# zouyunkai/MedicalSemSeg

Measured on AMD Instinct MI355X. Metric: 96^3 vols/sec fwd+bwd (train), higher is better.
Workload: dtype bf16; 1 GPU; UNet base (MONAI BasicUNet 32-32-64-128-256-32) 1->3cls, 96^3 patches, DiceCE + AdamW, per-GPU batch 2; global_batch=2, parallelism=dp1, grad_sync=none (single rank)

## Files before the change

### include/msseg.h

```cpp
#ifndef MSSEG_H_
#define MSSEG_H_

#include <stddef.h>
#include <stdint.h>

#ifdef __cplusplus
extern "C" {
#endif

#define MSSEG_ABI_VERSION 1

#define MSSEG_OK 0
#define MSSEG_EINVAL (-1)
#define MSSEG_ELAUNCH (-2)
#define MSSEG_EWORKSPACE (-3)

#define MSSEG_F32 0
#define MSSEG_BF16 1

typedef void* msseg_stream_t;

int msseg_abi_version(void);
const char* msseg_last_error(void);
int msseg_num_cus(void);
// ... 2 lines not shown
int msseg_ktimer_reset(void);
int msseg_ktimer_count(void);
int msseg_ktimer_get(int i, char* name, int cap, float* ms);

size_t msseg_packed_weight_bytes(int M, int T, int K, int cout_block, int dtype);
int msseg_pack_weights(const float* src, void* dst, int dtype, int M, int M0, int T, int K, int K0,
                       long long s_m1, long long s_m0, long long s_t, long long s_k1, long long s_k0,
                       int flip, int cout_block, msseg_stream_t stream);
typedef struct msseg_pack_job {
    const float* src;
    void* dst;
    long long s_m1, s_m0, s_t, s_k1, s_k0;
    long long total;
    int M, M0, T, K, K0, flip, cout_block, nkb;
} msseg_pack_job;
int msseg_pack_weights_batch(const msseg_pack_job* jobs_dev, int njobs, long long max_total, long long sum_total, int dtype,
                             msseg_stream_t stream);
int msseg_cout_block(int M);
int msseg_conv3d_k3_cout_block(int N, int D, int H, int W, int Cout);
int msseg_conv3d_k3_variant(int N, int D, int H, int W, int Cout);
int msseg_conv3d_k3_kernel(int N, int D, int H, int W, int Cin, int Cout, int dtype);

int msseg_conv3d_k3_fwd(const void* x, long long ldx, const void* wp, const float* bias, void* y, long long ldy,
                        int N, int D, int H, int W, int Cin, int Cout, float* stats ,
                        void* scratch, size_t scratch_bytes, int dtype, msseg_stream_t stream);
int msseg_conv3d_k3_fwd_accumulate(const void* x, long long ldx, const void* wp, void* y, long long ldy, int N, int D, int H,
                                   int W, int Cin, int Cout, float* stats, void* scratch, size_t scratch_bytes, int dtype,
                                   msseg_stream_t stream);
int msseg_conv3d_k3_dgrad_inbwd(const void* dy, long long lddy, const void* wp, void* da, long long ldda, int N, int D,
                                int H, int W, int Cin, int Cout, const void* yraw, long long ldyraw, const void* act,
                                long long ldact, const float* fwd_stats, float slope, float eps, float* red,
                                float* dgamma, float* dbeta, int accumulate, void* scratch, size_t scratch_bytes,
                                int dtype, msseg_stream_t stream);
int msseg_conv3d_k3s2_fwd(const void* x, long long ldx, const void* wp, const float* bias, void* y, long long ldy,
                          int N, int ID, int IH, int IW, int Cin, int Cout, int dtype, msseg_stream_t stream);
int msseg_zero_stuff2(const void* dy, long long lddy, void* out, long long ldo, int N, int OD, int OH, int OW, int ID,
                      int IH, int IW, int C, int dtype, msseg_stream_t stream);
int msseg_conv3d_stem_fwd(const void* x, long long ldx, const void* wp, const float* bias, void* y, long long ldy,
                          int N, int D, int H, int W, int Cout, float* stats, void* scratch, size_t scratch_bytes,
                          int dtype, msseg_stream_t stream);
int msseg_conv3d_stem_k1_fwd(const void* x, long long ldx, const void* wp, const float* bias, void* y, long long ldy,
                             int N, int D, int H, int W, int Cout, float* stats, void* scratch, size_t scratch_bytes,
                             int dtype, msseg_stream_t stream);
int msseg_conv3d_stem_norm_fwd(const void* x, long long ldx, const void* wp, const float* bias, const float* stats,
                               const float* gamma, const float* beta, float eps, float slope, void* y, long long ldy, int N,
                               int D, int H, int W, int Cout, int dtype, msseg_stream_t stream);
int msseg_conv3d_k1_fwd(const void* x, long long ldx, const void* wp, const float* bias, void* y, long long ldy,
                        long long NV, int Cin, int Cout, int dtype, msseg_stream_t stream);
int msseg_conv3d_k1_head_fwd(const void* x, long long ldx, const float* w, const float* bias, void* y, long long ldy,
                             long long NV, int Cin, int Cout, int dtype, msseg_stream_t stream);
int msseg_conv3d_k1_head_dgrad_inbwd(const void* dy, long long lddy, const float* w, void* da, long long ldda, int N,
                                     long long S, int C, int Cout, const void* yraw, long long ldyraw,
                                     const float* fwd_stats, const float* gamma, const float* beta, float slope, float eps,
                                     float* red, float* dgamma, float* dbeta, int accumulate, void* scratch,
                                     size_t scratch_bytes, int dtype, msseg_stream_t stream);
int msseg_conv3d_k1_head_norm_fwd(const void* x, long long ldx, const float* stats, const float* gamma, const float* beta,
                                  float slope, float eps, const float* w, const float* bias, void* y, long long ldy, int N,
                                  long long S, int Cin, int Cout, int dtype, msseg_stream_t stream);
int msseg_conv3d_k1_head_bwd_fused(const void* dy, long long lddy, const float* w, void* da, long long ldda, int N,
                                   long long S, int C, int Cout, const void* yraw, long long ldyraw, const float* fwd_stats,
                                   const float* gamma, const float* beta, float slope, float eps, float* red, float* dgamma,
                                   float* dbeta, int accumulate, float* dw, int dw_accumulate, void* scratch,
                                   size_t scratch_bytes, int dtype, msseg_stream_t stream);

int msseg_conv3d_gather_fwd(const void* x, long long ldx, const void* wp, const float* bias, void* y, long long ldy,
                            int N, int ID, int IH, int IW, int Cin, int Cout, int k, int s, int p, int dtype,
                            msseg_stream_t stream);
int msseg_deconv_k2s2_fwd(const void* x, long long ldx, const void* wp, const float* bias, void* y, long long ldy,
                          int N, int D, int H, int W, int Cin, int Cout, int dtype, msseg_stream_t stream);
int msseg_deconv_k2s2_bwd_data(const void* dy, long long lddy, const void* wp, void* dx, long long lddx,
                               int N, int D, int H, int W, int Cin, int Cout, int dtype, msseg_stream_t stream);
int msseg_deconv_k4s4_fwd(const void* x, long long ldx, const void* wp, const float* bias, void* y, long long ldy,
                          int N, int D, int H, int W, int Cin, int Cout, int dtype, msseg_stream_t stream);
// ... 74 lines not shown
int msseg_interp_trilinear_bwd(const void* dy, long long lddy, void* dx, long long lddx, int N, int ID, int IH, int IW, int OD,
                               int OH, int OW, int C, void* workspace, size_t workspace_bytes, int dtype, msseg_stream_t stream);
int msseg_kv_attention_fwd(const void* q, const void* kv, void* o, float* lse, int B, int N, int M, int heads, int head_dim,
                           float scale, int dtype, msseg_stream_t stream);
size_t msseg_kv_attention_bwd_workspace_bytes(int B, int N, int M, int heads, int head_dim);
int msseg_kv_attention_bwd(const void* q, const void* kv, const void* o, const float* lse, const void* dout, void* dq, void* dkv,
                           int B, int N, int M, int heads, int head_dim, float scale, void* workspace, size_t workspace_bytes,
                           int dtype, msseg_stream_t stream);
int msseg_scale_channels(const void* x, const float* scale, void* y, int N, long long S, int C, int dtype, msseg_stream_t stream);

size_t msseg_reduce_scratch_bytes(void);
int msseg_channel_stats(const void* x, long long ldx, float* stats, int N, long long S, int C, void* scratch,
                        size_t scratch_bytes, int dtype, msseg_stream_t stream);
int msseg_instnorm_act_fwd(const void* x, long long ldx, const float* stats, const float* gamma, const float* beta,
                           const void* residual, long long ldr, void* y, long long ldy, int N, long long S, int C,
                           float eps, float slope, int dtype, msseg_stream_t stream);
int msseg_instnorm_act_pool_fwd(const void* x, long long ldx, const float* stats, const float* gamma, const float* beta,
                                void* y, long long ldy, void* pooled, long long ldp, int N, int D, int H, int W, int C,
                                float eps, float slope, int dtype, msseg_stream_t stream);
int msseg_instnorm_act_poolbwd_reduce(const void* x, long long ldx, const float* stats, const float* gamma,
                                      const float* beta, const void* skip, long long lds, const void* g, long long ldg,
                                      void* da, long long ldda, float* red, float* dgamma, float* dbeta, int accumulate,
                                      int N, int D, int H, int W, int C, float eps, float slope, void* scratch,
                                      size_t scratch_bytes, int dtype, msseg_stream_t stream);
int msseg_instnorm_act_bwd_reduce(const void* x, long long ldx, const float* stats, const float* gamma,
                                  const float* beta, const void* y, long long ldy,
                                  const void* dy, long long lddy, float* red, float* dgamma, float* dbeta,
                                  int accumulate, int N, long long S, int C, float eps, float slope, void* scratch,
                                  size_t scratch_bytes, int dtype, msseg_stream_t stream);
int msseg_instnorm_act_bwd_apply(const void* x, long long ldx, const float* stats, const float* gamma,
                                 const float* beta, const void* y, long long ldy, const void* dy, long long lddy, const float* red, void* dx,
                                 long long lddx, void* dres, long long lddres, int N, long long S, int C, float eps,
                                 float slope, int dtype, msseg_stream_t stream);
int msseg_maxpool2_fwd(const void* x, long long ldx, void* y, long long ldy, int N, int D, int H, int W, int C,
                       int dtype, msseg_stream_t stream);
int msseg_maxpool2_bwd(const void* x, long long ldx, const void* dy, long long lddy, void* dx, long long lddx,
                       int N, int D, int H, int W, int C, int accumulate, int dtype, msseg_stream_t stream);
int msseg_ncdhw_to_ndhwc(const void* src, int src_dtype, void* dst, long long ldd, int dst_dtype, int N, int C,
                         long long S, msseg_stream_t stream);
int msseg_ndhwc_to_ncdhw(const void* src, long long lds, int src_dtype, void* dst, int dst_dtype, int N, int C,
                         long long S, msseg_stream_t stream);
int msseg_channel_sum(const void* x, long long ldx, float* out, long long rows, int C, int accumulate, void* scratch,
                      size_t scratch_bytes, int dtype, msseg_stream_t stream);
int msseg_add(const void* a, long long lda, const void* b, long long ldb, void* y, long long ldy, long long rows,
              int C, int dtype, msseg_stream_t stream);
int msseg_axpy_rows(const void* a, const void* b, const float* scale, void* y, int N, long long elems_per_sample, int dtype,
                    msseg_stream_t stream);


int msseg_window_attention_fwd(const void* qkv, const float* qkv_bias, const float* table, void* out, float* lse, int B,
                               int S, int H, int W, int C, int heads, int ws, int shift, int dtype,
                               msseg_stream_t stream);
int msseg_window_attention_bwd(const void* qkv, const float* qkv_bias, const float* table, const void* out,
                               const float* lse, const void* dout, void* dqkv, float* dtable, int B, int S, int H, int W,
                               int C, int heads, int ws, int shift, int dtype, msseg_stream_t stream);
size_t msseg_window_attention_bwd_workspace_bytes(int B, int S, int H, int W, int C, int heads, int ws, int shift, int dtype);
int msseg_window_attention_fwd2(const void* qkv, const float* qkv_bias, const float* table, void* out, float* lse, int B,
                                int S, int H, int W, int C, int heads, int ws, int shift, int bias_ws, int dtype,
                                msseg_stream_t stream);
int msseg_window_attention_bwd2(const void* qkv, const float* qkv_bias, const float* table, const void* out,
                                const float* lse, const void* dout, void* dqkv, float* dtable, int B, int S, int H, int W,
                                int C, int heads, int ws, int shift, int bias_ws, int dtype, void* workspace,
                                size_t workspace_bytes, msseg_stream_t stream);
int msseg_window_attention_bwd_ws(const void* qkv, const float* qkv_bias, const float* table, const void* out,
                                  const float* lse, const void* dout, void* dqkv, float* dtable, int B, int S, int H, int W,
                                  int C, int heads, int ws, int shift, int dtype, void* workspace, size_t workspace_bytes,
// ... 115 lines not shown
```

### medicalsemseg_amd/csrc/conv3d_k3_c48.hip

```cpp
#include "k3pp.h"

#include <stdlib.h>

#include <type_traits>

namespace {

constexpr int TD = 4, TH = 4, TW = 16;
constexpr int PD = TD + 2, PH = TH + 2, PW = TW + 2;
constexpr int HV = PD * PH * PW;
constexpr int VB = 96;
constexpr int ROWC = PW * 6;
constexpr int NCHUNK = HV * 6;
constexpr int NPIECE = (NCHUNK + 63) / 64;
constexpr int HALO_BYTES = NPIECE * 1024;
constexpr int NPW = (NPIECE + 3) / 4;
constexpr int NGRP = 14;
constexpr int NGRP_LDS = 10;
constexpr int NRES = (NGRP - NGRP_LDS) * 3;
constexpr int W_BYTES = NGRP_LDS * 3 * 1024;
constexpr int NMAX = 4;
constexpr int STAT_FLOATS = 8 * NMAX * 16 * 2;
constexpr int NTHREADS = 512;
constexpr int LDS_BYTES = W_BYTES + 2 * HALO_BYTES;
// ... 313 lines not shown
        float* wsp = p.stats_ws + ((long long)blockIdx.y * gridDim.x + blockIdx.x) * PN;
        for (int i = tid; i < PN; i += NTHREADS) {
            float s = 0.f;
#pragma unroll
            for (int wv = 0; wv < 8; ++wv) s += ldsS[wv * NMAX * 32 + i];
            wsp[i] = s;
        }
    }
}

int grid_x(const K3ppParams& p) {
    const int ncb = p.M / 16;
    const int tiles = p.N * ceil_div(p.D, TD) * ceil_div(p.H, TH) * ceil_div(p.W, TW);
    int gx = msseg_num_cus() / ncb;
    gx &= ~7;
    if (gx < 8) gx = 8;
    if (gx > tiles) gx = tiles;
    return gx;
}

template <int STATS, int TIMING = 0> int launch(const K3ppParams& p, hipStream_t stream) {
    const int lds = LDS_BYTES + (STATS ? STAT_FLOATS * 4 : 0);
    auto kern = k3c48_kernel<STATS, TIMING>;
    static msseg_lds_attr_once attr;
    if (!attr.ensure((const void*)kern, lds)) MSSEG_FAIL(MSSEG_ELAUNCH, "conv3d_k3_c48: cannot set dynamic LDS size %d", lds);
    const int ncb = p.M / 16, gx = grid_x(p);
    MSSEG_KTIMED("k3c48_kernel", stream, hipLaunchKernelGGL(kern, dim3(gx, ncb, 1), dim3(NTHREADS), lds, stream, p));
    MSSEG_CHECK_LAUNCH("conv3d_k3_c48");
    if (STATS != 0) {
        K3FinParams f{};
        f.ws = p.stats_ws; f.R = gx; f.N = p.N; f.coutb = 16; f.M = p.M; f.stats = p.stats;
        f.nb_stats = (STATS == 2) ? p.nb_stats : nullptr; f.nb_eps = p.nb_eps; f.nb_S = p.nb_S;
        f.nb_dgamma = p.nb_dgamma; f.nb_dbeta = p.nb_dbeta; f.nb_acc = p.nb_acc;
        return msseg_k3_stats_finalize(f, ncb, stream);
    }
    return MSSEG_OK;
}

}

bool msseg_k3c48_shape_ok(int N, int D, int H, int W, int M) {
    static const bool off = getenv("MSSEG_NO_K3C48") != nullptr || getenv("MSSEG_NO_K3PP") != nullptr;
    if (off) return false;
    if (M % 16 || M < 16 || M > 256 || N < 1 || N > NMAX) return false;
    const long long tiles = (long long)N * ceil_div(D, TD) * ceil_div(H, TH) * ceil_div(W, TW);
    if (tiles > 0x7fffffffLL) return false;
    if ((long long)(PD + 1) * H * W * 256 * 2 >= 0x7fffffffLL) return false;
    return tiles * (M / 16) >= 2LL * msseg_num_cus();
}

bool msseg_k3c48_eligible(const K3ppParams& p) {
    if (p.K != 48 || !msseg_k3c48_shape_ok(p.N, p.D, p.H, p.W, p.M)) return false;
    if ((p.ldx % 8) || p.ldx > 256 || (p.ldy % 4) || ((uintptr_t)p.x & 15) || ((uintptr_t)p.y & 7)) return false;
    if (p.bias && ((uintptr_t)p.bias & 15)) return false;
    if (p.nb_y && ((p.nb_ldy % 4) || (p.nb_lda % 4) || ((uintptr_t)p.nb_y & 7) || ((uintptr_t)p.nb_a & 7))) return false;
    return true;
}

int msseg_k3c48_launch(const K3ppParams& p, hipStream_t stream) {
    if (p.accumulate) {
        if (p.stats == nullptr || p.nb_y != nullptr) MSSEG_FAIL(MSSEG_EINVAL, "conv3d_k3_c48: accumulate mode comes with forward statistics");
        return launch<3>(p, stream);
    }
    static const bool timing = getenv("MSSEG_K3C48_TIMING") != nullptr;
    if (p.stats == nullptr) return timing ? launch<0, 1>(p, stream) : launch<0>(p, stream);
    if (p.nb_y == nullptr) return launch<1>(p, stream);
    return timing ? launch<2, 1>(p, stream) : launch<2>(p, stream);
// ... 6 lines not shown
```

### medicalsemseg_amd/csrc/conv3d_k3_pp.hip

```cpp
#include "k3pp.h"

#include <type_traits>

namespace {

constexpr int TD = 4, TH = 4, TW = 16;
constexpr int PD = TD + 2, PH = TH + 2, PW = TW + 2;
constexpr int HV = PD * PH * PW;
constexpr int PLANE = ((HV * 16 + 255) / 256) * 256;
constexpr int HALO_BYTES = 4 * PLANE;
constexpr int W_BYTES = 27 * 4 * 32 * 16;
constexpr int STAT_FLOATS = 8 * MSSEG_STATS_NMAX * 32 * 2;
constexpr int NTHREADS = 512;

__device__ u32x4_t g_zero_chunk;
__device__ unsigned long long g_k3pp_cycles[8];

MSSEG_DEVFN void glds16(const void* g, void* l) {
    __builtin_amdgcn_global_load_lds((const __attribute__((address_space(1))) void*)g,
                                     (__attribute__((address_space(3))) void*)l, 16, 0, 0);
}

struct TileCo { int n, d0, h0, w0; };

// ... 297 lines not shown

    if constexpr (STATS != 0) {
        flush_stats();
        __syncthreads();
        const int PN = p.N * 32 * 2;
        float* wsp = p.stats_ws + ((long long)blockIdx.y * gridDim.x + blockIdx.x) * PN;
        for (int i = tid; i < PN; i += NTHREADS) {
            float s = 0.f;
#pragma unroll
            for (int wv = 0; wv < 8; ++wv) s += ldsS[wv * MSSEG_STATS_NMAX * 64 + i];
            wsp[i] = s;
        }
    }
}

template <int STATS, int TIMING> int launch(const K3ppParams& p, hipStream_t stream) {
    const int lds = W_BYTES + 2 * HALO_BYTES + (STATS ? STAT_FLOATS * 4 : 0);
    auto kern = k3pp_kernel<STATS, TIMING>;
    static msseg_lds_attr_once attr;
    if (!attr.ensure((const void*)kern, lds)) MSSEG_FAIL(MSSEG_ELAUNCH, "conv3d_k3_pp: cannot set dynamic LDS size %d", lds);
    const int ncb = p.M / 32;
    const int tiles = p.N * ceil_div(p.D, TD) * ceil_div(p.H, TH) * ceil_div(p.W, TW);
    int gx = msseg_num_cus() / ncb;
    gx &= ~7;
    if (gx < 8) gx = 8;
    if (gx > tiles) gx = tiles;
    MSSEG_KTIMED("k3pp_kernel", stream, hipLaunchKernelGGL(kern, dim3(gx, ncb, 1), dim3(NTHREADS), lds, stream, p));
    MSSEG_CHECK_LAUNCH("conv3d_k3_pp");
    if (STATS != 0) {
        K3FinParams f{};
        f.ws = p.stats_ws; f.R = gx; f.N = p.N; f.coutb = 32; f.M = p.M; f.stats = p.stats;
        f.nb_stats = (STATS == 2) ? p.nb_stats : nullptr; f.nb_eps = p.nb_eps; f.nb_S = p.nb_S;
        f.nb_dgamma = p.nb_dgamma; f.nb_dbeta = p.nb_dbeta; f.nb_acc = p.nb_acc;
        return msseg_k3_stats_finalize(f, ncb, stream);
    }
    return MSSEG_OK;
}

}

bool msseg_k3pp_eligible(const K3ppParams& p) {
    static const bool off = getenv("MSSEG_NO_K3PP") != nullptr;
    if (off) return false;
    if (p.K != 32 || p.M % 32 || p.M > 256) return false;
    if ((p.ldx % 8) || (p.ldy % 4) || ((uintptr_t)p.x & 15) || ((uintptr_t)p.y & 7)) return false;
    if (p.bias && ((uintptr_t)p.bias & 15)) return false;
    if (p.stats && p.N > MSSEG_STATS_NMAX) return false;
    if (p.nb_y && ((p.nb_ldy % 4) || (p.nb_lda % 4) || ((uintptr_t)p.nb_y & 7) || ((uintptr_t)p.nb_a & 7))) return false;
    const long long tiles = (long long)p.N * ceil_div(p.D, TD) * ceil_div(p.H, TH) * ceil_div(p.W, TW);
    if (tiles > 0x7fffffffLL) return false;
    return tiles * (p.M / 32) >= 2LL * msseg_num_cus();
}

int msseg_k3pp_launch(const K3ppParams& p, hipStream_t stream) {
    static const bool timing = getenv("MSSEG_K3PP_TIMING") != nullptr;
    if (p.accumulate) {
        if (p.stats == nullptr || p.nb_y != nullptr) MSSEG_FAIL(MSSEG_EINVAL, "conv3d_k3_pp: accumulate mode comes with forward statistics");
        return launch<3, 0>(p, stream);
    }
    if (p.stats == nullptr) return timing ? launch<0, 1>(p, stream) : launch<0, 0>(p, stream);
    if (p.nb_y == nullptr) return timing ? launch<1, 1>(p, stream) : launch<1, 0>(p, stream);
    return launch<2, 0>(p, stream);
}

extern "C" int msseg_debug_k3pp_cycles(unsigned long long* out8) {
    return hipMemcpyFromSymbol(out8, HIP_SYMBOL(g_k3pp_cycles), 8 * sizeof(unsigned long long)) == hipSuccess ? 0 : -1;
}
// ... 1 lines not shown
```

### medicalsemseg_amd/csrc/elementwise.hip

```cpp
#include "common.h"

#include <stdarg.h>
#include <string.h>

static thread_local char g_err[512] = "";
void msseg_set_error(const char* fmt, ...) {
    va_list ap;
    va_start(ap, fmt);
    vsnprintf(g_err, sizeof(g_err), fmt, ap);
    va_end(ap);
}

extern "C" {
int msseg_abi_version(void) { return MSSEG_ABI_VERSION; }
const char* msseg_last_error(void) { return g_err; }
int msseg_num_cus(void) {
    static int cus = 0;
    if (cus == 0) {
        int dev = 0;
        hipDeviceProp_t prop;
        if (hipGetDevice(&dev) == hipSuccess && hipGetDeviceProperties(&prop, dev) == hipSuccess)
            cus = prop.multiProcessorCount;
        if (cus <= 0) cus = 256;
    }
    return cus;
}
}

namespace {

template <typename T> struct Chunk {
    static constexpr int EPC = DT<T>::EPC;
    float v[EPC];
// ... 282 lines not shown
    long long blocks = reduce_blocks(S, m.rows_par, N, C, nacc);
    const long long rpb = ceil_div_ll(S, blocks);
    blocks = ceil_div_ll(S, rpb);
    dim3 grid((unsigned)blocks, N);
    unsigned int* counter = (unsigned int*)scratch;
    float* ws = (float*)((unsigned char*)scratch + MSSEG_SCRATCH_COUNTER_BYTES);
    if (vec)
        hipLaunchKernelGGL((channel_stats_kernel<T, true>), grid, dim3(RED_THREADS), 0, st, (const T*)x, ldx, out, S, C,
                           m.groups, m.rows_par, rpb, nacc, accumulate, ws, counter);
    else
        hipLaunchKernelGGL((channel_stats_kernel<T, false>), grid, dim3(RED_THREADS), 0, st, (const T*)x, ldx, out, S, C,
                           m.groups, m.rows_par, rpb, nacc, accumulate, ws, counter);
    MSSEG_CHECK_LAUNCH("channel_stats");
    {
        FinalizeArgs a{ws, N, (int)blocks, C, nacc, nacc == 2 ? 0 : 1, out, nullptr, nullptr, accumulate};
        hipLaunchKernelGGL(channels_finalize_kernel, channels_finalize_grid(a), dim3(256), 0, st, a);
        MSSEG_CHECK_LAUNCH("channels_finalize");
    }
    return MSSEG_OK;
}

struct NormParams {
    const void* x; long long ldx;
    const float* stats; const float* gamma; const float* beta;
    const void* res; long long ldr;
    void* y; long long ldy;
    const void* dy; long long lddy;
    float* red;
    void* dx; long long lddx;
    void* dres; long long lddres;
    long long S; int C; float eps, slope;
    long long rows_per_block; int groups, rows_par;
    float* ws; unsigned int* counter; float* dgamma; float* dbeta; int accumulate;
};

MSSEG_DEVFN void mean_rstd(const float* stats, int n, int C, int c, long long S, float eps, float& mean, float& rstd) {
    const float inv = 1.0f / (float)S;
    const float s = stats[((long long)n * C + c) * 2 + 0], s2 = stats[((long long)n * C + c) * 2 + 1];
    mean = s * inv;
    float var = s2 * inv - mean * mean;
    var = var > 0.f ? var : 0.f;
    rstd = rsqrtf(var + eps);
}

template <typename T, bool VEC, int MODE>
__global__ __launch_bounds__(MODE == 1 ? RED_THREADS : 256) void instnorm_kernel(const NormParams p) {
    constexpr int W = VEC ? DT<T>::EPC : 1;
    __shared__ float red[(MODE == 1) ? RED_THREADS * 2 * W : 1];
    __shared__ int lflag;
    const int n = blockIdx.y;
    const int g = threadIdx.x % p.groups, rl = threadIdx.x / p.groups;
    const long long r0 = (long long)blockIdx.x * p.rows_per_block;
    long long r1 = r0 + p.rows_per_block;
    if (r1 > p.S) r1 = p.S;
    const T* xn = (const T*)p.x + (long long)n * p.S * p.ldx;
    const T* yn = (MODE != 0 && p.y != nullptr) ? (const T*)p.y + (long long)n * p.S * p.ldy : nullptr;
    T* yo = (MODE == 0) ? (T*)p.y + (long long)n * p.S * p.ldy : nullptr;
    const T* dyn = (MODE != 0) ? (const T*)p.dy + (long long)n * p.S * p.lddy : nullptr;
    const T* resn = (MODE == 0 && p.res) ? (const T*)p.res + (long long)n * p.S * p.ldr : nullptr;
    T* dxn = (MODE == 2) ? (T*)p.dx + (long long)n * p.S * p.lddx : nullptr;
    T* drn = (MODE == 2 && p.dres) ? (T*)p.dres + (long long)n * p.S * p.lddres : nullptr;
    const float invS = 1.0f / (float)p.S;

    for (int gbase = 0; gbase * W < p.C; gbase += p.groups) {
        const int gg = gbase + g;
        const bool act = gg * W < p.C;
        float mean[W], rstd[W], sc[W], sh[W], k0[W], k1[W], a0[W], a1[W];
#pragma unroll
        for (int e = 0; e < W; ++e) {
            const int c = act ? gg * W + e : 0;
            mean_rstd(p.stats, n, p.C, c, p.S, p.eps, mean[e], rstd[e]);
            const float ga = p.gamma ? p.gamma[c] : 1.f;
            sc[e] = rstd[e] * ga;
            sh[e] = (p.beta ? p.beta[c] : 0.f) - mean[e] * sc[e];
            a0[e] = a1[e] = 0.f;
            if constexpr (MODE == 2) {
                k0[e] = p.red[((long long)n * p.C + c) * 2 + 0] * invS;
                k1[e] = p.red[((long long)n * p.C + c) * 2 + 1] * invS;
            }
        }
        if (act && rl < p.rows_par) {
#pragma unroll 4
            for (long long r = r0 + rl; r < r1; r += p.rows_par) {
                float xv[W], o[W], yv[W], dv[W];
                if constexpr (VEC) {
                    Chunk<T> c; c.load(xn + r * p.ldx + gg * W);
#pragma unroll
                    for (int e = 0; e < W; ++e) xv[e] = c.v[e];
                } else {
                    xv[0] = DT<T>::ld(xn + r * p.ldx + gg);
                }
                if constexpr (MODE == 0) {
                    float rv[W];
#pragma unroll
                    for (int e = 0; e < W; ++e) rv[e] = 0.f;
                    if (resn) {
                        if constexpr (VEC) {
                            Chunk<T> c; c.load(resn + r * p.ldr + gg * W);
#pragma unroll
                            for (int e = 0; e < W; ++e) rv[e] = c.v[e];
                        } else {
                            rv[0] = DT<T>::ld(resn + r * p.ldr + gg);
                        }
                    }
#pragma unroll
                    for (int e = 0; e < W; ++e) {
                        const float z = xv[e] * sc[e] + sh[e] + rv[e];
                        o[e] = z > 0.f ? z : z * p.slope;
                    }
                    if constexpr (VEC) {
                        Chunk<T> c;
// ... 55 lines not shown
            __syncthreads();
#pragma unroll
            for (int e = 0; e < W; ++e) {
                red[(threadIdx.x * W + e) * 2 + 0] = a0[e];
                red[(threadIdx.x * W + e) * 2 + 1] = a1[e];
            }
            __syncthreads();
            block_rows_reduce<W>(red, p.groups, p.rows_par, g, rl, act);
            if (act && rl == 0) {
                const int kmax = p.rows_par < RED_STAGE2 ? p.rows_par : RED_STAGE2;
#pragma unroll
                for (int e = 0; e < W; ++e) {
                    float a = 0.f, b = 0.f;
                    for (int k = 0; k < kmax; ++k) {
                        a += red[((k * p.groups + g) * W + e) * 2 + 0];
                        b += red[((k * p.groups + g) * W + e) * 2 + 1];
                    }
                    const int c = gg * W + e;
                    float* wsb = p.ws + ((long long)n * gridDim.x + blockIdx.x) * p.C * 2;
                    wsb[c * 2 + 0] = a;
                    wsb[c * 2 + 1] = b;
                }
            }
        }
    }
}

struct NormPoolParams {
    const void* x; long long ldx;
    const float* stats; const float* gamma; const float* beta;
    void* y; long long ldy;
    void* pooled; long long ldp;
    int N, D, H, W, C; float eps, slope;
};

template <typename T>
__global__ __launch_bounds__(256) void instnorm_pool_fwd_kernel(const NormPoolParams p) {
    constexpr int WD = DT<T>::EPC;
    const int OD = p.D / 2, OH = p.H / 2, OW = p.W / 2;
    const unsigned ug = (unsigned)(p.C / WD);
    const unsigned total = (unsigned)((long long)p.N * OD * OH * OW * ug);
    const long long S = (long long)p.D * p.H * p.W;
    for (unsigned i = blockIdx.x * 256u + threadIdx.x; i < total; i += gridDim.x * 256u) {
        unsigned t = i / ug;
        const int g = (int)(i - t * ug);
        unsigned t2 = t / (unsigned)OW;
        const int ow = (int)(t - t2 * (unsigned)OW);
        t = t2 / (unsigned)OH;
        const int oh = (int)(t2 - t * (unsigned)OH);
        const int n = (int)(t / (unsigned)OD);
        const int od = (int)(t - (unsigned)n * (unsigned)OD);
        float sc[WD], sh[WD], best[WD];
#pragma unroll
        for (int e = 0; e < WD; ++e) {
            const int c = g * WD + e;
            float mean, rstd;
            mean_rstd(p.stats, n, p.C, c, S, p.eps, mean, rstd);
            sc[e] = rstd * (p.gamma ? p.gamma[c] : 1.f);
            sh[e] = (p.beta ? p.beta[c] : 0.f) - mean * sc[e];
            best[e] = -INFINITY;
        }
        Chunk<T> in[8];
#pragma unroll
        for (int k = 0; k < 8; ++k) {
            const long long vox = (((long long)n * p.D + 2 * od + (k >> 2)) * p.H + 2 * oh + ((k >> 1) & 1)) * p.W + 2 * ow + (k & 1);
            in[k].load((const T*)p.x + vox * p.ldx + g * WD);
        }
#pragma unroll
        for (int k = 0; k < 8; ++k) {
            const long long vox = (((long long)n * p.D + 2 * od + (k >> 2)) * p.H + 2 * oh + ((k >> 1) & 1)) * p.W + 2 * ow + (k & 1);
            Chunk<T> o;
#pragma unroll
            for (int e = 0; e < WD; ++e) {
                const float z = in[k].v[e] * sc[e] + sh[e];
                const float a = (float)(T)(z > 0.f ? z : z * p.slope);
                o.v[e] = a;
                if (a > best[e] || a != a) best[e] = a;
            }
            o.store((T*)p.y + vox * p.ldy + g * WD);
        }
        Chunk<T> b;
#pragma unroll
        for (int e = 0; e < WD; ++e) b.v[e] = best[e];
        const long long ovox = (((long long)n * OD + od) * OH + oh) * OW + ow;
        b.store((T*)p.pooled + ovox * p.ldp + g * WD);
    }
}

struct NormPoolBwdParams {
    const void* x; long long ldx;
// ... 214 lines not shown
            if (act && rl == 0) {
                const int kmax = p.rows_par < RED_STAGE2 ? p.rows_par : RED_STAGE2;
#pragma unroll
                for (int e = 0; e < WD; ++e) {
                    float a = 0.f, b = 0.f;
                    for (int k = 0; k < kmax; ++k) {
                        a += red[((k * p.groups + g) * WD + e) * 2 + 0];
                        b += red[((k * p.groups + g) * WD + e) * 2 + 1];
                    }
                    wsb[(gg * WD + e) * NPER + 2 * round + 0] = a;
                    wsb[(gg * WD + e) * NPER + 2 * round + 1] = b;
                }
            }
        }
    }
}

template <typename T, int MODE> int launch_norm(NormParams& p, int N, bool vec, hipStream_t st) {
    constexpr int NTHR = MODE == 1 ? RED_THREADS : 256;
    const RowMap m = row_map(p.C, vec ? DT<T>::EPC : 1, NTHR);
    p.groups = m.groups; p.rows_par = m.rows_par;
    long long blocks;
    if (MODE == 1) {
        blocks = reduce_blocks(p.S, m.rows_par, N, p.C, 2);
    } else {
        blocks = ceil_div_ll(p.S, (long long)m.rows_par * 4);
        const long long cap = (long long)msseg_num_cus() * 8 / (N > 0 ? N : 1);
        if (blocks > cap) blocks = cap;
        if (blocks < 1) blocks = 1;
    }
    p.rows_per_block = ceil_div_ll(p.S, blocks);
    blocks = ceil_div_ll(p.S, p.rows_per_block);
    dim3 grid((unsigned)blocks, N);
    if (vec) hipLaunchKernelGGL((instnorm_kernel<T, true, MODE>), grid, dim3(NTHR), 0, st, p);
    else hipLaunchKernelGGL((instnorm_kernel<T, false, MODE>), grid, dim3(NTHR), 0, st, p);
    MSSEG_CHECK_LAUNCH("instnorm");
    if (MODE == 1) {
        FinalizeArgs a{p.ws, N, (int)blocks, p.C, 2, 2, p.red, p.dbeta, p.dgamma, p.accumulate};
        hipLaunchKernelGGL(channels_finalize_kernel, channels_finalize_grid(a), dim3(256), 0, st, a);
        MSSEG_CHECK_LAUNCH("channels_finalize");
    }
    return MSSEG_OK;
}

template <typename T, bool VEC, bool BWD>
__global__ __launch_bounds__(256) void maxpool2_kernel(const T* __restrict__ x, long long ldx, const T* __restrict__ dy,
                                                       long long lddy, T* __restrict__ out, long long ldo, int N, int D,
                                                       int H, int W, int C, int accumulate) {
    constexpr int WD = VEC ? DT<T>::EPC : 1;
    const int OD = D / 2, OH = H / 2, OW = W / 2;
    const int groups = (C + WD - 1) / WD;
    const unsigned total = (unsigned)((long long)N * OD * OH * OW * groups);
    for (unsigned i = blockIdx.x * 256u + threadIdx.x; i < total; i += gridDim.x * 256u) {
        const unsigned ug = (unsigned)groups;
        unsigned t = i / ug;
        const int g = (int)(i - t * ug);
        unsigned t2 = t / (unsigned)OW;
        const int ow = (int)(t - t2 * (unsigned)OW);
        t = t2 / (unsigned)OH;
        const int oh = (int)(t2 - t * (unsigned)OH);
        const int n = (int)(t / (unsigned)OD);
        const int od = (int)(t - (unsigned)n * (unsigned)OD);
        float best[WD];
        int arg[WD];
#pragma unroll
        for (int e = 0; e < WD; ++e) { best[e] = -INFINITY; arg[e] = 0; }
// ... 455 lines not shown
    if (!scratch || ((uintptr_t)scratch & 255) || bytes < msseg_reduce_scratch_bytes())
        MSSEG_FAIL(MSSEG_EWORKSPACE, "%s: needs a zero-initialised, 256-byte aligned scratch of %zu bytes", who,
                   msseg_reduce_scratch_bytes());
    return MSSEG_OK;
}

int msseg_layernorm_param_grad(const void* x, long long ldx, const float* mean, const float* rstd, const void* dy,
                               long long lddy, float* dgamma, float* dbeta, int accumulate, long long rows, int C,
                               void* scratch, size_t scratch_bytes, int dtype, msseg_stream_t stream) {
    if (!x || !mean || !rstd || !dy || !dgamma || !dbeta || rows < 1 || C < 1)
        MSSEG_FAIL(MSSEG_EINVAL, "layernorm_param_grad: bad args");
    if (int rc = scratch_ok(scratch, scratch_bytes, "layernorm_param_grad")) return rc;
    DISPATCH_T(dtype,
               return launch_ln_param_grad<float>(x, ldx, dy, lddy, mean, rstd, dgamma, dbeta, accumulate, rows, C, scratch, (hipStream_t)stream),
               return launch_ln_param_grad<bf16_t>(x, ldx, dy, lddy, mean, rstd, dgamma, dbeta, accumulate, rows, C, scratch, (hipStream_t)stream));
}

int msseg_channel_stats(const void* x, long long ldx, float* stats, int N, long long S, int C, void* scratch,
                        size_t scratch_bytes, int dtype, msseg_stream_t stream) {
    if (!x || !stats || N < 1 || S < 1 || C < 1 || ldx < C) MSSEG_FAIL(MSSEG_EINVAL, "channel_stats: bad args");
    if (int rc = scratch_ok(scratch, scratch_bytes, "channel_stats")) return rc;
    DISPATCH_T(dtype, return launch_stats<float>(x, ldx, stats, N, S, C, 2, 0, scratch, (hipStream_t)stream),
               return launch_stats<bf16_t>(x, ldx, stats, N, S, C, 2, 0, scratch, (hipStream_t)stream));
}

int msseg_channel_sum(const void* x, long long ldx, float* out, long long rows, int C, int accumulate, void* scratch,
                      size_t scratch_bytes, int dtype, msseg_stream_t stream) {
    if (!x || !out || rows < 1 || C < 1 || ldx < C) MSSEG_FAIL(MSSEG_EINVAL, "channel_sum: bad args");
    if (int rc = scratch_ok(scratch, scratch_bytes, "channel_sum")) return rc;
    DISPATCH_T(dtype, return launch_stats<float>(x, ldx, out, 1, rows, C, 1, accumulate, scratch, (hipStream_t)stream),
               return launch_stats<bf16_t>(x, ldx, out, 1, rows, C, 1, accumulate, scratch, (hipStream_t)stream));
}

int msseg_instnorm_act_fwd(const void* x, long long ldx, const float* stats, const float* gamma, const float* beta,
                           const void* residual, long long ldr, void* y, long long ldy, int N, long long S, int C,
                           float eps, float slope, int dtype, msseg_stream_t stream) {
    if (!x || !stats || !y || N < 1 || S < 1 || C < 1) MSSEG_FAIL(MSSEG_EINVAL, "instnorm_act_fwd: bad args");
    NormParams p{};
    p.x = x; p.ldx = ldx; p.stats = stats; p.gamma = gamma; p.beta = beta; p.res = residual; p.ldr = ldr;
    p.y = y; p.ldy = ldy; p.S = S; p.C = C; p.eps = eps; p.slope = slope;
    const int esz = dtype == MSSEG_F32 ? 4 : 2;
    const bool vec = vec_ok(x, ldx, C, esz) && vec_ok(y, ldy, C, esz) && (!residual || vec_ok(residual, ldr, C, esz));
    DISPATCH_T(dtype, return (launch_norm<float, 0>(p, N, vec, (hipStream_t)stream)),
               return (launch_norm<bf16_t, 0>(p, N, vec, (hipStream_t)stream)));
}

int msseg_conv3d_k1_head_fwd(const void* x, long long ldx, const float* w, const float* bias, void* y, long long ldy,
                             long long NV, int Cin, int Cout, int dtype, msseg_stream_t stream) {
    if (!x || !w || !y || NV < 1) MSSEG_FAIL(MSSEG_EINVAL, "conv3d_k1_head: bad args");
    const int esz = dtype == MSSEG_F32 ? 4 : 2;
    if (dtype != MSSEG_F32 && dtype != MSSEG_BF16) MSSEG_FAIL(MSSEG_EINVAL, "conv3d_k1_head: bad dtype");
    if (Cout < 1 || Cout > 4 || Cin < 1 || Cin > 64 || !vec_ok(x, ldx, Cin, esz) || ldy < Cout)
        MSSEG_FAIL(MSSEG_EINVAL, "conv3d_k1_head: needs 1 <= Cout <= 4, Cin <= 64 in 16-byte chunks (got %d -> %d)", Cin, Cout);
    const int g = grid_for(NV, 1);
#define HEAD(T_, C_) hipLaunchKernelGGL((conv1x1_head_kernel<T_, C_>), dim3(g), dim3(256), 0, (hipStream_t)stream, \
                                        (const T_*)x, ldx, w, bias, (T_*)y, ldy, NV, Cin)
#define HEAD_C(T_) do { if (Cout == 1) HEAD(T_, 1); else if (Cout == 2) HEAD(T_, 2); else if (Cout == 3) HEAD(T_, 3); else HEAD(T_, 4); } while (0)
    DISPATCH_T(dtype, HEAD_C(float), HEAD_C(bf16_t));
#undef HEAD_C
#undef HEAD
    MSSEG_CHECK_LAUNCH("conv3d_k1_head");
    return MSSEG_OK;
}

static int head_bwd_impl(const void* dy, long long lddy, const float* w, void* da, long long ldda, int N, long long S,
                         int C, int Cout, const void* yraw, long long ldyraw, const float* fwd_stats, const float* gamma,
                         const float* beta, float slope, float eps, float* red, float* dgamma, float* dbeta, int accumulate,
                         float* dw, int dw_accumulate, void* scratch, size_t scratch_bytes, int dtype,
                         msseg_stream_t stream) {
    if (!dy || !w || !da || !yraw || !fwd_stats || !red || N < 1 || S < 1)
        MSSEG_FAIL(MSSEG_EINVAL, "conv3d_k1_head_dgrad_inbwd: bad args");
// ... 43 lines not shown
                                   float* dbeta, int accumulate, float* dw, int dw_accumulate, void* scratch,
                                   size_t scratch_bytes, int dtype, msseg_stream_t stream) {
    if (!dw) MSSEG_FAIL(MSSEG_EINVAL, "conv3d_k1_head_bwd_fused: dw is required");
    return head_bwd_impl(dy, lddy, w, da, ldda, N, S, C, Cout, yraw, ldyraw, fwd_stats, gamma, beta, slope, eps, red, dgamma,
                         dbeta, accumulate, dw, dw_accumulate, scratch, scratch_bytes, dtype, stream);
}

int msseg_conv3d_k1_head_norm_fwd(const void* x, long long ldx, const float* stats, const float* gamma, const float* beta,
                                  float slope, float eps, const float* w, const float* bias, void* y, long long ldy, int N,
                                  long long S, int Cin, int Cout, int dtype, msseg_stream_t stream) {
    if (!x || !stats || !w || !y || N < 1 || S < 1) MSSEG_FAIL(MSSEG_EINVAL, "conv3d_k1_head_norm: bad args");
    const int esz = dtype == MSSEG_F32 ? 4 : 2;
    if (dtype != MSSEG_F32 && dtype != MSSEG_BF16) MSSEG_FAIL(MSSEG_EINVAL, "conv3d_k1_head_norm: bad dtype");
    if ((gamma == nullptr) != (beta == nullptr)) MSSEG_FAIL(MSSEG_EINVAL, "conv3d_k1_head_norm: gamma/beta go together");
    if (Cout < 1 || Cout > 4 || Cin < 1 || Cin > 64 || !vec_ok(x, ldx, Cin, esz) || ldy < Cout)
        MSSEG_FAIL(MSSEG_EINVAL, "conv3d_k1_head_norm: needs 1 <= Cout <= 4, Cin <= 64 in 16-byte chunks (got %d -> %d)", Cin, Cout);
    long long gx = ceil_div_ll(S, 256);
    const long long cap = (long long)msseg_num_cus() * 16 / N + 1;
    if (gx > cap) gx = cap;
    dim3 grid((unsigned)gx, N);
#define HEADN(T_, C_) hipLaunchKernelGGL((conv1x1_head_norm_kernel<T_, C_>), grid, dim3(256), 0, (hipStream_t)stream, \
                                         (const T_*)x, ldx, stats, gamma, beta, slope, eps, w, bias, (T_*)y, ldy, S, Cin)
#define HEADN_C(T_) do { if (Cout == 1) HEADN(T_, 1); else if (Cout == 2) HEADN(T_, 2); else if (Cout == 3) HEADN(T_, 3); else HEADN(T_, 4); } while (0)
    DISPATCH_T(dtype, HEADN_C(float), HEADN_C(bf16_t));
#undef HEADN_C
#undef HEADN
    MSSEG_CHECK_LAUNCH("conv3d_k1_head_norm");
    return MSSEG_OK;
}

int msseg_instnorm_act_pool_fwd(const void* x, long long ldx, const float* stats, const float* gamma, const float* beta,
                                void* y, long long ldy, void* pooled, long long ldp, int N, int D, int H, int W, int C,
                                float eps, float slope, int dtype, msseg_stream_t stream) {
    if (!x || !stats || !y || !pooled || N < 1 || D < 2 || H < 2 || W < 2 || C < 1)
        MSSEG_FAIL(MSSEG_EINVAL, "instnorm_act_pool_fwd: bad args");
    if ((D | H | W) & 1) MSSEG_FAIL(MSSEG_EINVAL, "instnorm_act_pool_fwd: odd spatial size %dx%dx%d", D, H, W);
    const int esz = dtype == MSSEG_F32 ? 4 : 2;
    if (dtype != MSSEG_F32 && dtype != MSSEG_BF16) MSSEG_FAIL(MSSEG_EINVAL, "instnorm_act_pool_fwd: bad dtype");
    if (!(vec_ok(x, ldx, C, esz) && vec_ok(y, ldy, C, esz) && vec_ok(pooled, ldp, C, esz)))
        MSSEG_FAIL(MSSEG_EINVAL, "instnorm_act_pool_fwd: needs 16-byte aligned rows and a channel count multiple of %d", 16 / esz);
    const long long total = (long long)N * (D / 2) * (H / 2) * (W / 2) * (C / (16 / esz));
    if (total >= 0x7fffffffLL) MSSEG_FAIL(MSSEG_EINVAL, "instnorm_act_pool_fwd: too many elements");
    NormPoolParams p{x, ldx, stats, gamma, beta, y, ldy, pooled, ldp, N, D, H, W, C, eps, slope};
    const int g = grid_for(total, 1);
    DISPATCH_T(dtype, hipLaunchKernelGGL(instnorm_pool_fwd_kernel<float>, dim3(g), dim3(256), 0, (hipStream_t)stream, p),
               hipLaunchKernelGGL(instnorm_pool_fwd_kernel<bf16_t>, dim3(g), dim3(256), 0, (hipStream_t)stream, p));
    MSSEG_CHECK_LAUNCH("instnorm_act_pool_fwd");
    return MSSEG_OK;
}

int msseg_instnorm_act_poolbwd_reduce(const void* x, long long ldx, const float* stats, const float* gamma,
                                      const float* beta, const void* skip, long long lds, const void* g, long long ldg,
                                      void* da, long long ldda, float* red, float* dgamma, float* dbeta, int accumulate,
                                      int N, int D, int H, int W, int C, float eps, float slope, void* scratch,
                                      size_t scratch_bytes, int dtype, msseg_stream_t stream) {
    if (!x || !stats || !skip || !g || !da || !red || N < 1 || D < 2 || H < 2 || W < 2 || C < 1)
        MSSEG_FAIL(MSSEG_EINVAL, "instnorm_act_poolbwd_reduce: bad args");
    if ((D | H | W) & 1) MSSEG_FAIL(MSSEG_EINVAL, "instnorm_act_poolbwd_reduce: odd spatial size %dx%dx%d", D, H, W);
    if (dtype != MSSEG_F32 && dtype != MSSEG_BF16) MSSEG_FAIL(MSSEG_EINVAL, "instnorm_act_poolbwd_reduce: bad dtype");
    if (int rc = scratch_ok(scratch, scratch_bytes, "instnorm_act_poolbwd_reduce")) return rc;
    const int esz = dtype == MSSEG_F32 ? 4 : 2;
    if (!(vec_ok(x, ldx, C, esz) && vec_ok(skip, lds, C, esz) && vec_ok(g, ldg, C, esz) && vec_ok(da, ldda, C, esz)))
        MSSEG_FAIL(MSSEG_EINVAL, "instnorm_act_poolbwd_reduce: needs 16-byte aligned rows and a channel count multiple of %d",
                   16 / esz);
    NormPoolBwdParams p{x, ldx, stats, gamma, beta, skip, lds, g, ldg, da, ldda, N, D, H, W, C, eps, slope, 0, 0, 0, nullptr};
    p.ws = (float*)((unsigned char*)scratch + MSSEG_SCRATCH_COUNTER_BYTES);
    const RowMap m = row_map(C, 16 / esz, RED_THREADS);
    p.groups = m.groups; p.rows_par = m.rows_par;
    const long long cells = (long long)(D / 2) * (H / 2) * (W / 2);
    long long blocks = reduce_blocks(cells * 8, m.rows_par, N, C, 2);
    p.cells_per_block = ceil_div_ll(cells, blocks);
    blocks = ceil_div_ll(cells, p.cells_per_block);
    dim3 grid((unsigned)blocks, N);
    DISPATCH_T(dtype,
               hipLaunchKernelGGL(instnorm_poolbwd_reduce_kernel<float>, grid, dim3(RED_THREADS), 0, (hipStream_t)stream, p),
               hipLaunchKernelGGL(instnorm_poolbwd_reduce_kernel<bf16_t>, grid, dim3(RED_THREADS), 0, (hipStream_t)stream, p));
    MSSEG_CHECK_LAUNCH("instnorm_act_poolbwd_reduce");
    FinalizeArgs a{p.ws, N, (int)blocks, C, 2, 2, red, dbeta, dgamma, accumulate};
    hipLaunchKernelGGL(channels_finalize_kernel, channels_finalize_grid(a), dim3(256), 0, (hipStream_t)stream, a);
    MSSEG_CHECK_LAUNCH("channels_finalize");
    return MSSEG_OK;
}

int msseg_instnorm_act_bwd_reduce(const void* x, long long ldx, const float* stats, const float* gamma,
                                  const float* beta, const void* y, long long ldy,
                                  const void* dy, long long lddy, float* red, float* dgamma, float* dbeta,
                                  int accumulate, int N, long long S, int C, float eps, float slope, void* scratch,
                                  size_t scratch_bytes, int dtype, msseg_stream_t stream) {
    if (!x || !stats || !dy || !red) MSSEG_FAIL(MSSEG_EINVAL, "instnorm_act_bwd_reduce: null pointer");
    if (int rc = scratch_ok(scratch, scratch_bytes, "instnorm_act_bwd_reduce")) return rc;
    NormParams p{};
    p.counter = (unsigned int*)scratch;
    p.ws = (float*)((unsigned char*)scratch + MSSEG_SCRATCH_COUNTER_BYTES);
    p.dgamma = dgamma; p.dbeta = dbeta; p.accumulate = accumulate;
    p.x = x; p.ldx = ldx; p.stats = stats; p.gamma = gamma; p.beta = beta; p.y = (void*)y; p.ldy = ldy; p.dy = dy; p.lddy = lddy; p.red = red;
    p.S = S; p.C = C; p.eps = eps; p.slope = slope;
    const int esz = dtype == MSSEG_F32 ? 4 : 2;
    const bool vec = vec_ok(x, ldx, C, esz) && vec_ok(y, ldy, C, esz) && vec_ok(dy, lddy, C, esz);
    DISPATCH_T(dtype, return (launch_norm<float, 1>(p, N, vec, (hipStream_t)stream)),
               return (launch_norm<bf16_t, 1>(p, N, vec, (hipStream_t)stream)));
}

int msseg_instnorm_act_bwd_apply(const void* x, long long ldx, const float* stats, const float* gamma,
                                 const float* beta, const void* y, long long ldy, const void* dy, long long lddy, const float* red, void* dx,
                                 long long lddx, void* dres, long long lddres, int N, long long S, int C, float eps,
                                 float slope, int dtype, msseg_stream_t stream) {
    if (!x || !stats || !dy || !red || !dx) MSSEG_FAIL(MSSEG_EINVAL, "instnorm_act_bwd_apply: null pointer");
    NormParams p{};
    p.x = x; p.ldx = ldx; p.stats = stats; p.gamma = gamma; p.beta = beta; p.y = (void*)y; p.ldy = ldy; p.dy = dy; p.lddy = lddy;
    p.red = (float*)red; p.dx = dx; p.lddx = lddx; p.dres = dres; p.lddres = lddres;
    p.S = S; p.C = C; p.eps = eps; p.slope = slope;
    const int esz = dtype == MSSEG_F32 ? 4 : 2;
    const bool vec = vec_ok(x, ldx, C, esz) && vec_ok(y, ldy, C, esz) && vec_ok(dy, lddy, C, esz) &&
                     vec_ok(dx, lddx, C, esz) && (!dres || vec_ok(dres, lddres, C, esz));
    DISPATCH_T(dtype, return (launch_norm<float, 2>(p, N, vec, (hipStream_t)stream)),
               return (launch_norm<bf16_t, 2>(p, N, vec, (hipStream_t)stream)));
}

int msseg_maxpool2_fwd(const void* x, long long ldx, void* y, long long ldy, int N, int D, int H, int W, int C,
                       int dtype, msseg_stream_t stream) {
    if (!x || !y || D < 2 || H < 2 || W < 2 || C < 1) MSSEG_FAIL(MSSEG_EINVAL, "maxpool2_fwd: bad args");
    const int esz = dtype == MSSEG_F32 ? 4 : 2;
    const bool vec = vec_ok(x, ldx, C, esz) && vec_ok(y, ldy, C, esz);
    const long long total = (long long)N * (D / 2) * (H / 2) * (W / 2) * ceil_div(C, vec ? 16 / esz : 1);
    if (total >= 0x7fffffffLL) MSSEG_FAIL(MSSEG_EINVAL, "maxpool2_fwd: too many elements");
    const int g = grid_for(total, 1);
#define MP_F(T_, V_) hipLaunchKernelGGL((maxpool2_kernel<T_, V_, false>), dim3(g), dim3(256), 0, (hipStream_t)stream, \
                                        (const T_*)x, ldx, (const T_*)nullptr, 0LL, (T_*)y, ldy, N, D, H, W, C, 0)
    DISPATCH_T(dtype, if (vec) MP_F(float, true); else MP_F(float, false),
               if (vec) MP_F(bf16_t, true); else MP_F(bf16_t, false));
#undef MP_F
    MSSEG_CHECK_LAUNCH("maxpool2_fwd");
    return MSSEG_OK;
}

int msseg_maxpool2_bwd(const void* x, long long ldx, const void* dy, long long lddy, void* dx, long long lddx, int N,
                       int D, int H, int W, int C, int accumulate, int dtype, msseg_stream_t stream) {
    if (!x || !dy || !dx || D < 2 || H < 2 || W < 2 || C < 1) MSSEG_FAIL(MSSEG_EINVAL, "maxpool2_bwd: bad args");
    const int esz = dtype == MSSEG_F32 ? 4 : 2;
    const bool vec = vec_ok(x, ldx, C, esz) && vec_ok(dy, lddy, C, esz) && vec_ok(dx, lddx, C, esz);
    const long long total = (long long)N * (D / 2) * (H / 2) * (W / 2) * ceil_div(C, vec ? 16 / esz : 1);
// ... 132 lines not shown
```

### medicalsemseg_amd/csrc/igemm_fwd.hip

```cpp
#include "common.h"
#include "k3pp.h"

#include <stdlib.h>

#include <type_traits>

namespace {

enum { SRC_DIRECT = 0, SRC_GATHER = 1, SRC_DECONV_BWD = 2 };
enum { EPI_STORE = 0, EPI_DECONV = 1 };

struct IgemmParams {
    const void* x;
    long long ldx;
    const void* wp;
    const float* bias;
    void* y;
    long long ldy;
    int N, D, H, W;
    int ID, IH, IW;
    int OD, OH, OW;
    int K, M, NKB;
    int tiles_d, tiles_h, tiles_w;
    int ntiles;
    int cin, k, s, p;
    int creal;
    int vec_store;
    int rel32_ok;
    int cout_block;
    float* stats;
    float* stats_ws;
    unsigned int* counter;
    const void* nb_y; long long nb_ldy;
    const void* nb_a; long long nb_lda;
    const float* nb_stats;
    float nb_slope, nb_eps; long long nb_S;
    float* nb_dgamma; float* nb_dbeta; int nb_acc;
};

template <typename T, int NTAPS, int SRC, int EPI, int TD, int TH, int TW, int WAVES, int NT, int STRIDE = 1, int NSL = 1>
struct IgemmCfg {
    static constexpr int EPC = DT<T>::EPC;
    static constexpr int CB = 4 * EPC;
    static constexpr int PAD = (NTAPS == 27) ? 1 : 0;
    static constexpr int PD = (TD - 1) * STRIDE + 1 + 2 * PAD, PH = (TH - 1) * STRIDE + 1 + 2 * PAD,
                         PW = (TW - 1) * STRIDE + 1 + 2 * PAD;
    static constexpr int HV = PD * PH * PW;
    static constexpr int TV = TD * TH * TW;
    static constexpr int MT = TV / 16 / WAVES;
    static constexpr int NTHREADS = WAVES * 64;
    static constexpr int COUTB = NT * 16;
    static constexpr int PLANE = ((HV * 16 + 255) / 256) * 256;
    static constexpr int A_BYTES = ((4 * PLANE + 64 + 255) / 256) * 256;
    static constexpr int BT = NTAPS / NSL;
    static constexpr int B_BYTES = BT * 4 * COUTB * 16;
    static_assert(NTAPS % NSL == 0, "tap slices must divide the taps");
    static constexpr int STAT_FLOATS = MSSEG_STATS_NMAX * COUTB * 2;
    static constexpr int STAT_BYTES = (EPI == EPI_STORE) ? (STAT_FLOATS + WAVES * COUTB * 2) * 4 + 256 : 0;
    static constexpr int LDS_BYTES = A_BYTES + B_BYTES + STAT_BYTES;
    static_assert(TV % (16 * WAVES) == 0, "tile must split into 16-voxel MFMA tiles per wave");
};

MSSEG_DEVFN int aoff(int q, int plane) { return q * plane + (q >> 1) * 32; }

// ... 500 lines not shown
                                    const float dz = av[e] > 0.f ? da : da * p.nb_slope;
                                    st[j][e] += dz;
                                    st2[j][e] += dz * yv[e];
                                }
                            }
                        }
                    }
                }
            }
        }
        if (kb == p.NKB - 1 && ks == NSL - 1 && p.vec_store) { ptc = tc; pend_valid = true; }
        mark(6);
        tile = ntile; kb = nkb; ks = nks; tc = ntc;
    }
    store_pending();
    if constexpr (DIAG == 5) {
        if (blockIdx.x == 0 && tid == 0) {
#pragma unroll
            for (int k = 0; k < 8; ++k) g_phase_cycles[k] = ph[k];
        }
    }
    if constexpr (EPI == EPI_STORE) {
        if (do_stats) {
            if (cur_n >= 0) flush_stats(cur_n);
            __syncthreads();
            const int PN = p.N * COUTB * 2;
            float* wsp = p.stats_ws + ((long long)blockIdx.y * gridDim.x + blockIdx.x) * PN;
            for (int i = tid; i < PN; i += NTHREADS) wsp[i] = spart[i];
        }
    }
}

__global__ __launch_bounds__(256) void k3_stats_finalize_kernel(const K3FinParams f) {
    __shared__ __attribute__((aligned(16))) float fin[256 * 4 + 8 * 48 * 2];
    const int tid = threadIdx.x;
    const int L = f.N * f.coutb * 2;
    const int cbase = blockIdx.x * f.coutb;
    if (f.nb_stats == nullptr) {
        const int n = blockIdx.y, Ls = f.coutb * 2;
        block_rows_sum<256>(f.ws + (long long)blockIdx.x * f.R * L + n * Ls, f.R, Ls, fin, L);
        const float* tot = fin + 256 * 4;
        for (int i = tid; i < Ls; i += 256) {
            const int cl = i >> 1, k = i & 1;
            if (cbase + cl < f.M) f.stats[((long long)n * f.M + cbase + cl) * 2 + k] = tot[i];
        }
        return;
    }
    block_rows_sum<256>(f.ws + (long long)blockIdx.x * f.R * L, f.R, L, fin);
    const float* tot = fin + 256 * 4;
    if (tid < f.coutb && cbase + tid < f.M) {
        const int cg = cbase + tid;
        float g0 = 0.f, g1 = 0.f;
        const float inv = 1.0f / (float)f.nb_S;
        for (int nn = 0; nn < f.N; ++nn) {
            const float a = tot[(nn * f.coutb + tid) * 2], b0 = tot[(nn * f.coutb + tid) * 2 + 1];
            const float fs = f.nb_stats[((long long)nn * f.M + cg) * 2], fs2 = f.nb_stats[((long long)nn * f.M + cg) * 2 + 1];
            const float mean = fs * inv;
            float var = fs2 * inv - mean * mean;
            var = var > 0.f ? var : 0.f;
            const float b2 = rsqrtf(var + f.nb_eps) * (b0 - mean * a);
            g0 += a;
            g1 += b2;
            f.stats[((long long)nn * f.M + cg) * 2 + 0] = a;
            f.stats[((long long)nn * f.M + cg) * 2 + 1] = b2;
        }
        if (f.nb_dgamma != nullptr) {
            f.nb_dbeta[cg] = f.nb_acc ? f.nb_dbeta[cg] + g0 : g0;
            f.nb_dgamma[cg] = f.nb_acc ? f.nb_dgamma[cg] + g1 : g1;
        }
    }
}

template <typename T, int NTAPS, int SRC, int EPI, int TD, int TH, int TW, int WAVES, int NT, int STRIDE = 1, int NSL = 1, int DIAG = 0>
int launch_cfg(IgemmParams& p, hipStream_t stream) {
    using C = IgemmCfg<T, NTAPS, SRC, EPI, TD, TH, TW, WAVES, NT, STRIDE, NSL>;
    p.tiles_d = ceil_div(p.D, TD);
    p.tiles_h = ceil_div(p.H, TH);
    p.tiles_w = ceil_div(p.W, TW);
    const long long nt = (long long)p.N * p.tiles_d * p.tiles_h * p.tiles_w;
    if (nt > 0x7fffffffLL) MSSEG_FAIL(MSSEG_EINVAL, "igemm: too many tiles");
    p.ntiles = (int)nt;
    p.NKB = ceil_div(p.K, C::CB);
    p.vec_store = ((((uintptr_t)p.y) % (4 * sizeof(T))) == 0 && (p.ldy % 4) == 0) ? 1 : 0;
    {
        const long long xh = STRIDE == 1 ? p.H : p.IH, xw = STRIDE == 1 ? p.W : p.IW;
        p.rel32_ok = ((long long)(C::PD + 1) * xh * xw * p.ldx < 0x7fffffffLL) ? 1 : 0;
    }
    auto kern = igemm_fwd_kernel<T, NTAPS, SRC, EPI, TD, TH, TW, WAVES, NT, STRIDE, NSL, DIAG>;
    static msseg_lds_attr_once attr;
    if (!attr.ensure((const void*)kern, C::LDS_BYTES)) MSSEG_FAIL(MSSEG_ELAUNCH, "igemm: cannot set dynamic LDS size %d", C::LDS_BYTES);
    const int ncb = ceil_div(p.M, C::COUTB);
    const int wg_per_cu = (C::LDS_BYTES > 80 * 1024) ? 1 : ((C::LDS_BYTES > 40 * 1024) ? 2 : 4);
    int gx = msseg_num_cus() * wg_per_cu / (ncb > 1 ? 1 : 1);
    if (gx > p.ntiles) gx = p.ntiles;
    if (gx < 1) gx = 1;
    dim3 grid(gx, ncb, 1);
    static const char* const kt_name = NTAPS != 27 ? "igemm_fwd_kernel<flat>"
                                       : (TD * TH * TW == 512 ? "igemm_fwd_kernel<27,4x8x16>"
                                          : (TD * TH * TW == 128 ? "igemm_fwd_kernel<27,4x4x8>" : "igemm_fwd_kernel<27,2x4x8>"));
    MSSEG_KTIMED(kt_name, stream, hipLaunchKernelGGL(kern, grid, dim3(C::NTHREADS), C::LDS_BYTES, stream, p));
    MSSEG_CHECK_LAUNCH("igemm_fwd");
    if (EPI == EPI_STORE && p.stats != nullptr) {
        K3FinParams f{};
        f.ws = p.stats_ws; f.R = gx; f.N = p.N; f.coutb = C::COUTB; f.M = p.M; f.stats = p.stats;
        f.nb_stats = p.nb_y ? p.nb_stats : nullptr; f.nb_eps = p.nb_eps; f.nb_S = p.nb_S;
        f.nb_dgamma = p.nb_dgamma; f.nb_dbeta = p.nb_dbeta; f.nb_acc = p.nb_acc;
        return msseg_k3_stats_finalize(f, ncb, stream);
    }
    return MSSEG_OK;
}

template <typename T, int NTAPS, int SRC, int EPI, int TD, int TH, int TW, int WAVES, int STRIDE = 1, int NSL = 1>
int launch_nt(IgemmParams& p, hipStream_t stream) {
    const int cb = p.cout_block ? p.cout_block : msseg_cout_block(p.M);
    switch (cb) {
        case 16: return launch_cfg<T, NTAPS, SRC, EPI, TD, TH, TW, WAVES, 1, STRIDE, NSL>(p, stream);
        case 32: return launch_cfg<T, NTAPS, SRC, EPI, TD, TH, TW, WAVES, 2, STRIDE, NSL>(p, stream);
        case 48: return launch_cfg<T, NTAPS, SRC, EPI, TD, TH, TW, WAVES, 3, STRIDE, NSL>(p, stream);
    }
    MSSEG_FAIL(MSSEG_EINVAL, "igemm: bad cout block %d", cb);
}

static void k3_plan(int N, int D, int H, int W, int M, int* cfg, int* cb) {
    const int mn = D < H ? (D < W ? D : W) : (H < W ? H : W);
    const int std_cb = msseg_cout_block(M);
    {
        static const char* force = getenv("MSSEG_K3_FORCE");
        if (force && mn < 32 && std_cb == 32) {
            *cfg = force[0] - '0';
            *cb = atoi(force + 2);
            return;
        }
    }
    const long long want = (long long)msseg_num_cus() * 3 / 4;
    auto wgs = [&](int td, int th, int tw, int c) {
        return (long long)N * ceil_div(D, td) * ceil_div(H, th) * ceil_div(W, tw) * ceil_div(M, c);
    };
    if (mn >= 32 && wgs(4, 8, 16, std_cb) >= want) {
        *cfg = 0;
        *cb = (std_cb == 48) ? 32 : std_cb;
// ... 21 lines not shown
                    case '4': return launch_cfg<T, 27, SRC_DIRECT, EPI_STORE, 4, 8, 16, 8, 2, 1, 1, 4>(p, stream);
                    case '5': return launch_cfg<T, 27, SRC_DIRECT, EPI_STORE, 4, 8, 16, 8, 2, 1, 1, 5>(p, stream);
                }
            }
        }
        if (old_big || cb == 48) return launch_nt<T, 27, SRC_DIRECT, EPI_STORE, 4, 8, 16, 8>(p, stream);
        return launch_nt<T, 27, SRC_DIRECT, EPI_STORE, 2, 8, 16, 4, 1, 3>(p, stream);
    }
    if (cfg == 1) return launch_nt<T, 27, SRC_DIRECT, EPI_STORE, 4, 4, 8, 4>(p, stream);
    return launch_nt<T, 27, SRC_DIRECT, EPI_STORE, 2, 4, 8, 4>(p, stream);
}

template <typename T, int SRC, int EPI> int launch_flat(IgemmParams& p, hipStream_t stream) {
    return launch_nt<T, 1, SRC, EPI, 1, 1, 256, 4>(p, stream);
}

int check_common(const void* x, long long ldx, const void* wp, const void* y, long long ldy, int dtype, int esz) {
    if (!x || !wp || !y) MSSEG_FAIL(MSSEG_EINVAL, "igemm: null pointer");
    if (dtype != MSSEG_F32 && dtype != MSSEG_BF16) MSSEG_FAIL(MSSEG_EINVAL, "igemm: bad dtype %d", dtype);
    if (((uintptr_t)x | (uintptr_t)wp) & 15) MSSEG_FAIL(MSSEG_EINVAL, "igemm: x/wp must be 16-byte aligned");
    if ((ldx * esz) % 16) MSSEG_FAIL(MSSEG_EINVAL, "igemm: ldx*elem must be a multiple of 16 bytes");
    (void)ldy;
    return MSSEG_OK;
}

}

int msseg_k3_stats_finalize(const K3FinParams& f, int ncb, hipStream_t stream) {
    hipLaunchKernelGGL(k3_stats_finalize_kernel, dim3(ncb, f.nb_stats ? 1 : f.N), dim3(256), 0, stream, f);
    MSSEG_CHECK_LAUNCH("k3_stats_finalize");
    return MSSEG_OK;
}

extern "C" int msseg_debug_phase_cycles(unsigned long long* out8) {
    return hipMemcpyFromSymbol(out8, HIP_SYMBOL(g_phase_cycles), 8 * sizeof(unsigned long long)) == hipSuccess ? 0 : -1;
}

extern "C" {

int msseg_cout_block(int M) {
    if (M <= 16) return 16;
    if (M % 32 == 0) return 32;
    if (M % 48 == 0) return 48;
    return 32;
}

int msseg_conv3d_k3_cout_block(int N, int D, int H, int W, int Cout) {
    int cfg, cb;
    k3_plan(N, D, H, W, Cout, &cfg, &cb);
    return cb;
}

int msseg_conv3d_k3_variant(int N, int D, int H, int W, int Cout) {
    int cfg, cb;
    k3_plan(N, D, H, W, Cout, &cfg, &cb);
    return cfg;
}

int msseg_conv3d_k3_kernel(int N, int D, int H, int W, int Cin, int Cout, int dtype) {
    int cfg, cb;
    if (dtype == MSSEG_BF16 && Cin == 48 && msseg_k3c48_shape_ok(N, D, H, W, Cout)) return 4;
    k3_plan(N, D, H, W, Cout, &cfg, &cb);
    if (dtype == MSSEG_BF16 && cb == 32) {
        K3ppParams pp{};
        pp.x = (const void*)256; pp.y = (void*)256; pp.ldx = Cin; pp.ldy = Cout;
        pp.N = N; pp.D = D; pp.H = H; pp.W = W; pp.K = Cin; pp.M = Cout;
        if ((Cin % 8) == 0 && (Cout % 4) == 0 && msseg_k3pp_eligible(pp)) return 3;
    }
    return cfg;
}

static int k3_fwd_impl(const void* x, long long ldx, const void* wp, const float* bias, void* y, long long ldy, int N,
                       int D, int H, int W, int Cin, int Cout, float* stats, void* scratch, size_t scratch_bytes,
                       const void* nb_y, long long nb_ldy, const void* nb_a, long long nb_lda, const float* nb_stats,
                       float nb_slope, float nb_eps, float* nb_dgamma, float* nb_dbeta, int nb_acc, int dtype,
                       msseg_stream_t stream);

int msseg_conv3d_k3_fwd(const void* x, long long ldx, const void* wp, const float* bias, void* y, long long ldy,
                        int N, int D, int H, int W, int Cin, int Cout, float* stats, void* scratch,
                        size_t scratch_bytes, int dtype, msseg_stream_t stream) {
    return k3_fwd_impl(x, ldx, wp, bias, y, ldy, N, D, H, W, Cin, Cout, stats, scratch, scratch_bytes, nullptr, 0, nullptr,
                       0, nullptr, 0.f, 0.f, nullptr, nullptr, 0, dtype, stream);
}

int msseg_conv3d_k3_fwd_accumulate(const void* x, long long ldx, const void* wp, void* y, long long ldy, int N, int D, int H,
                                   int W, int Cin, int Cout, float* stats, void* scratch, size_t scratch_bytes, int dtype,
                                   msseg_stream_t stream) {
    if (!x || !wp || !y || !stats) MSSEG_FAIL(MSSEG_EINVAL, "conv3d_k3_fwd_accumulate: null pointer");
    if (dtype != MSSEG_BF16 || N < 1 || N > MSSEG_STATS_NMAX) MSSEG_FAIL(MSSEG_EINVAL, "conv3d_k3_fwd_accumulate: bf16, N <= %d", MSSEG_STATS_NMAX);
    if (!scratch || ((uintptr_t)scratch & 255) || scratch_bytes < msseg_reduce_scratch_bytes())
        MSSEG_FAIL(MSSEG_EWORKSPACE, "conv3d_k3_fwd_accumulate: needs the reduce scratch of %zu bytes", msseg_reduce_scratch_bytes());
    K3ppParams pp{};
    pp.x = x; pp.ldx = ldx; pp.wp = wp; pp.y = y; pp.ldy = ldy;
    pp.N = N; pp.D = D; pp.H = H; pp.W = W; pp.K = Cin; pp.M = Cout;
    pp.stats = stats; pp.counter = (unsigned int*)scratch;
    pp.stats_ws = (float*)((unsigned char*)scratch + MSSEG_SCRATCH_COUNTER_BYTES);
    pp.accumulate = 1;
    if (Cin == 48) {
        if (!msseg_k3c48_eligible(pp))
            MSSEG_FAIL(MSSEG_EINVAL, "conv3d_k3_fwd_accumulate: 48 input channels need a shape and operands the 48-channel "
                                     "kernel takes (msseg_conv3d_k3_kernel() == 4, 16-byte aligned x, N <= 4)");
        return msseg_k3c48_launch(pp, (hipStream_t)stream);
    }
    if (!msseg_k3pp_eligible(pp))
        MSSEG_FAIL(MSSEG_EINVAL, "conv3d_k3_fwd_accumulate: only shapes of the ping-pong kernel (32 input channels, Cout %% 32 == 0, "
                                 "large grids; msseg_conv3d_k3_kernel() == 3)");
    return msseg_k3pp_launch(pp, (hipStream_t)stream);
}

int msseg_conv3d_k3_dgrad_inbwd(const void* dy, long long lddy, const void* wp, void* da, long long ldda, int N, int D,
                                int H, int W, int Cin, int Cout, const void* yraw, long long ldyraw, const void* act,
                                long long ldact, const float* fwd_stats, float slope, float eps, float* red,
                                float* dgamma, float* dbeta, int accumulate, void* scratch, size_t scratch_bytes,
                                int dtype, msseg_stream_t stream) {
    if (!yraw || !act || !fwd_stats || !red) MSSEG_FAIL(MSSEG_EINVAL, "conv3d_k3_dgrad_inbwd: null pointer");
    if ((dgamma == nullptr) != (dbeta == nullptr)) MSSEG_FAIL(MSSEG_EINVAL, "conv3d_k3_dgrad_inbwd: dgamma/dbeta go together");
    const int esz = dtype == MSSEG_F32 ? 4 : 2;
    if (Cout % 4 || (ldyraw % 4) || (ldact % 4) || ((uintptr_t)yraw % (4 * esz)) || ((uintptr_t)act % (4 * esz)))
        MSSEG_FAIL(MSSEG_EINVAL, "conv3d_k3_dgrad_inbwd: channel count / strides must be multiples of 4");
    return k3_fwd_impl(dy, lddy, wp, nullptr, da, ldda, N, D, H, W, Cin, Cout, red, scratch, scratch_bytes, yraw, ldyraw,
                       act, ldact, fwd_stats, slope, eps, dgamma, dbeta, accumulate, dtype, stream);
}

static int k3_fwd_impl(const void* x, long long ldx, const void* wp, const float* bias, void* y, long long ldy, int N,
                       int D, int H, int W, int Cin, int Cout, float* stats, void* scratch, size_t scratch_bytes,
                       const void* nb_y, long long nb_ldy, const void* nb_a, long long nb_lda, const float* nb_stats,
                       float nb_slope, float nb_eps, float* nb_dgamma, float* nb_dbeta, int nb_acc, int dtype,
                       msseg_stream_t stream) {
    const int esz = dtype == MSSEG_F32 ? 4 : 2;
    int rc = check_common(x, ldx, wp, y, ldy, dtype, esz);
    if (rc) return rc;
    if (N < 1 || D < 1 || H < 1 || W < 1 || Cin < 1 || Cout < 1) MSSEG_FAIL(MSSEG_EINVAL, "conv3d_k3: bad shape");
    if (Cin % (16 / esz)) MSSEG_FAIL(MSSEG_EINVAL, "conv3d_k3: Cin=%d must be a multiple of %d (use conv3d_gather)", Cin, 16 / esz);
    if (ldx < Cin || ldy < Cout) MSSEG_FAIL(MSSEG_EINVAL, "conv3d_k3: ld smaller than channels");
    IgemmParams p{};
    p.x = x; p.ldx = ldx; p.wp = wp; p.bias = bias; p.y = y; p.ldy = ldy;
    p.N = N; p.D = D; p.H = H; p.W = W; p.K = Cin; p.M = Cout;
    if (stats) {
        if (N > MSSEG_STATS_NMAX) MSSEG_FAIL(MSSEG_EINVAL, "conv3d_k3: fused statistics need N <= %d", MSSEG_STATS_NMAX);
        if (Cout > 64 * 16) MSSEG_FAIL(MSSEG_EINVAL, "conv3d_k3: fused statistics need Cout <= 1024 (one counter per cout block)");
        if (!scratch || ((uintptr_t)scratch & 255) || scratch_bytes < msseg_reduce_scratch_bytes())
            MSSEG_FAIL(MSSEG_EWORKSPACE, "conv3d_k3: fused statistics need a zero-initialised scratch of %zu bytes",
                       msseg_reduce_scratch_bytes());
        p.stats = stats;
        p.counter = (unsigned int*)scratch;
        p.stats_ws = (float*)((unsigned char*)scratch + MSSEG_SCRATCH_COUNTER_BYTES);
        p.nb_y = nb_y; p.nb_ldy = nb_ldy; p.nb_a = nb_a; p.nb_lda = nb_lda; p.nb_stats = nb_stats;
        p.nb_slope = nb_slope; p.nb_eps = nb_eps; p.nb_S = (long long)D * H * W;
        p.nb_dgamma = nb_dgamma; p.nb_dbeta = nb_dbeta; p.nb_acc = nb_acc;
    }
    if (dtype == MSSEG_BF16) {
        K3ppParams pp{};
        pp.x = x; pp.ldx = ldx; pp.wp = wp; pp.bias = bias; pp.y = y; pp.ldy = ldy;
        pp.N = N; pp.D = D; pp.H = H; pp.W = W; pp.K = Cin; pp.M = Cout;
        pp.stats = p.stats; pp.stats_ws = p.stats_ws; pp.counter = p.counter;
        pp.nb_y = p.nb_y; pp.nb_ldy = p.nb_ldy; pp.nb_a = p.nb_a; pp.nb_lda = p.nb_lda; pp.nb_stats = p.nb_stats;
        pp.nb_slope = p.nb_slope; pp.nb_eps = p.nb_eps; pp.nb_S = p.nb_S;
        pp.nb_dgamma = p.nb_dgamma; pp.nb_dbeta = p.nb_dbeta; pp.nb_acc = p.nb_acc;
        if (Cin == 48 && msseg_k3c48_shape_ok(N, D, H, W, Cout)) {
            if (!msseg_k3c48_eligible(pp))
                MSSEG_FAIL(MSSEG_EINVAL, "conv3d_k3: 48-input-channel layer on a large grid needs 16-byte aligned x, 8-byte "
                                         "aligned y and ldx <= 256");
            return msseg_k3c48_launch(pp, (hipStream_t)stream);
        }
        int cfg, cb;
        k3_plan(N, D, H, W, Cout, &cfg, &cb);
        if (cb == 32 && msseg_k3pp_eligible(pp)) return msseg_k3pp_launch(pp, (hipStream_t)stream);
    }
    return dtype == MSSEG_F32 ? launch_k3<float>(p, (hipStream_t)stream) : launch_k3<bf16_t>(p, (hipStream_t)stream);
}

int msseg_conv3d_k3s2_fwd(const void* x, long long ldx, const void* wp, const float* bias, void* y, long long ldy,
                          int N, int ID, int IH, int IW, int Cin, int Cout, int dtype, msseg_stream_t stream) {
    const int esz = dtype == MSSEG_F32 ? 4 : 2;
    int rc = check_common(x, ldx, wp, y, ldy, dtype, esz);
    if (rc) return rc;
    if (N < 1 || ID < 1 || IH < 1 || IW < 1 || Cin < 1 || Cout < 1) MSSEG_FAIL(MSSEG_EINVAL, "conv3d_k3s2: bad shape");
    if (Cin % (16 / esz)) MSSEG_FAIL(MSSEG_EINVAL, "conv3d_k3s2: Cin=%d must be a multiple of %d", Cin, 16 / esz);
    IgemmParams p{};
    p.x = x; p.ldx = ldx; p.wp = wp; p.bias = bias; p.y = y; p.ldy = ldy;
    p.N = N; p.ID = ID; p.IH = IH; p.IW = IW;
    p.D = (ID - 1) / 2 + 1; p.H = (IH - 1) / 2 + 1; p.W = (IW - 1) / 2 + 1;
    p.K = Cin; p.M = Cout;
    return dtype == MSSEG_F32 ? launch_nt<float, 27, SRC_DIRECT, EPI_STORE, 2, 4, 8, 4, 2>(p, (hipStream_t)stream)
                              : launch_nt<bf16_t, 27, SRC_DIRECT, EPI_STORE, 2, 4, 8, 4, 2>(p, (hipStream_t)stream);
}

int msseg_conv3d_stem_norm_fwd(const void* x, long long ldx, const void* wp, const float* bias, const float* stats,
                               const float* gamma, const float* beta, float eps, float slope, void* y, long long ldy, int N,
                               int D, int H, int W, int Cout, int dtype, msseg_stream_t stream) {
    if (!x || !wp || !y || !stats || N < 1 || D < 1 || H < 1 || W < 1) MSSEG_FAIL(MSSEG_EINVAL, "conv3d_stem_norm: bad args");
// ... 20 lines not shown
    p.N = 1; p.D = 1; p.H = 1; p.W = (int)NV; p.K = Cin; p.M = Cout;
    return dtype == MSSEG_F32 ? launch_flat<float, SRC_DIRECT, EPI_STORE>(p, (hipStream_t)stream)
                              : launch_flat<bf16_t, SRC_DIRECT, EPI_STORE>(p, (hipStream_t)stream);
}

int msseg_conv3d_gather_fwd(const void* x, long long ldx, const void* wp, const float* bias, void* y, long long ldy,
                            int N, int ID, int IH, int IW, int Cin, int Cout, int k, int s, int pd, int dtype,
                            msseg_stream_t stream) {
    const int esz = dtype == MSSEG_F32 ? 4 : 2;
    if (!x || !wp || !y) MSSEG_FAIL(MSSEG_EINVAL, "conv3d_gather: null pointer");
    if (dtype != MSSEG_F32 && dtype != MSSEG_BF16) MSSEG_FAIL(MSSEG_EINVAL, "conv3d_gather: bad dtype");
    if (k < 1 || s < 1 || pd < 0 || Cin < 1) MSSEG_FAIL(MSSEG_EINVAL, "conv3d_gather: bad kernel geometry");
    const int OD = (ID + 2 * pd - k) / s + 1, OH = (IH + 2 * pd - k) / s + 1, OW = (IW + 2 * pd - k) / s + 1;
    if (OD < 1 || OH < 1 || OW < 1) MSSEG_FAIL(MSSEG_EINVAL, "conv3d_gather: empty output");
    const long long NV = (long long)N * OD * OH * OW;
    if (NV > 0x7fffffffLL) MSSEG_FAIL(MSSEG_EINVAL, "conv3d_gather: too many voxels");
    if (msseg_stem_eligible(dtype, Cin, Cout, k, s, pd, ldx, ldy, y)) {
        StemParams sp{};
        sp.x = x; sp.ldx = ldx; sp.wp = wp; sp.bias = bias; sp.y = y; sp.ldy = ldy;
        sp.N = N; sp.D = ID; sp.H = IH; sp.W = IW; sp.M = Cout; sp.taps = k == 1 ? 1 : 27;
        return msseg_stem_fwd_launch(sp, (hipStream_t)stream);
    }
    IgemmParams p{};
    p.x = x; p.ldx = ldx; p.wp = wp; p.bias = bias; p.y = y; p.ldy = ldy;
    p.N = 1; p.D = 1; p.H = 1; p.W = (int)NV; p.K = Cin * k * k * k; p.M = Cout;
    p.ID = ID; p.IH = IH; p.IW = IW; p.OD = OD; p.OH = OH; p.OW = OW;
    p.cin = Cin; p.k = k; p.s = s; p.p = pd;
    return dtype == MSSEG_F32 ? launch_flat<float, SRC_GATHER, EPI_STORE>(p, (hipStream_t)stream)
                              : launch_flat<bf16_t, SRC_GATHER, EPI_STORE>(p, (hipStream_t)stream);
}

static int stem_fwd_taps(const void* x, long long ldx, const void* wp, const float* bias, void* y, long long ldy, int N, int D,
                         int H, int W, int Cout, float* stats, void* scratch, size_t scratch_bytes, int dtype, int taps,
                         msseg_stream_t stream);

int msseg_conv3d_stem_fwd(const void* x, long long ldx, const void* wp, const float* bias, void* y, long long ldy,
                          int N, int D, int H, int W, int Cout, float* stats, void* scratch, size_t scratch_bytes,
                          int dtype, msseg_stream_t stream) {
    return stem_fwd_taps(x, ldx, wp, bias, y, ldy, N, D, H, W, Cout, stats, scratch, scratch_bytes, dtype, 27, stream);
}

int msseg_conv3d_stem_k1_fwd(const void* x, long long ldx, const void* wp, const float* bias, void* y, long long ldy,
                             int N, int D, int H, int W, int Cout, float* stats, void* scratch, size_t scratch_bytes,
                             int dtype, msseg_stream_t stream) {
    return stem_fwd_taps(x, ldx, wp, bias, y, ldy, N, D, H, W, Cout, stats, scratch, scratch_bytes, dtype, 1, stream);
}

static int stem_fwd_taps(const void* x, long long ldx, const void* wp, const float* bias, void* y, long long ldy, int N, int D,
                         int H, int W, int Cout, float* stats, void* scratch, size_t scratch_bytes, int dtype, int taps,
                         msseg_stream_t stream) {
    if (!x || !wp || (!y && !stats) || N < 1 || D < 1 || H < 1 || W < 1) MSSEG_FAIL(MSSEG_EINVAL, "conv3d_stem: bad args");
    if (!msseg_stem_eligible(dtype, 1, Cout, 3, 1, 1, ldx, y ? ldy : 4, y))
        MSSEG_FAIL(MSSEG_EINVAL, "conv3d_stem: bf16, Cout a multiple of 32 or 48 (<= 256), 8-byte aligned output rows only");
    StemParams sp{};
    sp.x = x; sp.ldx = ldx; sp.wp = wp; sp.bias = bias; sp.y = y; sp.ldy = ldy;
    sp.N = N; sp.D = D; sp.H = H; sp.W = W; sp.M = Cout; sp.taps = taps;
    if (stats) {
        if (N > MSSEG_STATS_NMAX) MSSEG_FAIL(MSSEG_EINVAL, "conv3d_stem: fused statistics need N <= %d", MSSEG_STATS_NMAX);
        if (!scratch || ((uintptr_t)scratch & 255) || scratch_bytes < msseg_reduce_scratch_bytes())
            MSSEG_FAIL(MSSEG_EWORKSPACE, "conv3d_stem: fused statistics need a scratch of %zu bytes", msseg_reduce_scratch_bytes());
        sp.stats = stats;
        sp.stats_ws = (float*)((unsigned char*)scratch + MSSEG_SCRATCH_COUNTER_BYTES);
    }
    return msseg_stem_fwd_launch(sp, (hipStream_t)stream);
}

int msseg_deconv_k2s2_fwd(const void* x, long long ldx, const void* wp, const float* bias, void* y, long long ldy,
                          int N, int D, int H, int W, int Cin, int Cout, int dtype, msseg_stream_t stream) {
    const int esz = dtype == MSSEG_F32 ? 4 : 2;
    int rc = check_common(x, ldx, wp, y, ldy, dtype, esz);
    if (rc) return rc;
    if (Cin % (16 / esz) || Cout % 4) MSSEG_FAIL(MSSEG_EINVAL, "deconv_k2s2: Cin %% %d and Cout %% 4 must be 0", 16 / esz);
    const long long NV = (long long)N * D * H * W;
    if (NV < 1 || NV > 0x7fffffffLL / 8) MSSEG_FAIL(MSSEG_EINVAL, "deconv_k2s2: bad voxel count");
    if (msseg_deconv2_fast_eligible(dtype, Cin, Cout, x, ldx, y, ldy, bias))
        return msseg_deconv2_fwd_launch(x, ldx, wp, bias, y, ldy, N, D, H, W, Cin, Cout, (hipStream_t)stream);
    if (msseg_deconv2g_fwd_eligible(dtype, Cin, Cout, x, ldx, y, ldy, bias))
        return msseg_deconv2g_fwd_launch(x, ldx, wp, bias, y, ldy, N, D, H, W, Cin, Cout, (hipStream_t)stream);
    IgemmParams p{};
    p.x = x; p.ldx = ldx; p.wp = wp; p.bias = bias; p.y = y; p.ldy = ldy;
    p.N = 1; p.D = 1; p.H = 1; p.W = (int)NV; p.K = Cin; p.M = 8 * Cout;
    p.OD = D; p.OH = H; p.OW = W; p.creal = Cout;
    return dtype == MSSEG_F32 ? launch_flat<float, SRC_DIRECT, EPI_DECONV>(p, (hipStream_t)stream)
                              : launch_flat<bf16_t, SRC_DIRECT, EPI_DECONV>(p, (hipStream_t)stream);
}

int msseg_deconv_k2s2_bwd_data(const void* dy, long long lddy, const void* wp, void* dx, long long lddx,
                               int N, int D, int H, int W, int Cin, int Cout, int dtype, msseg_stream_t stream) {
    const int esz = dtype == MSSEG_F32 ? 4 : 2;
    int rc = check_common(dy, lddy, wp, dx, lddx, dtype, esz);
    if (rc) return rc;
    if (Cout % (16 / esz)) MSSEG_FAIL(MSSEG_EINVAL, "deconv_k2s2_bwd_data: Cout %% %d must be 0", 16 / esz);
    const long long NV = (long long)N * D * H * W;
    if (NV < 1 || NV > 0x7fffffffLL / 8) MSSEG_FAIL(MSSEG_EINVAL, "deconv_k2s2_bwd_data: bad voxel count");
    if (msseg_deconv2_fast_eligible(dtype, Cin, Cout, dx, lddx, dy, lddy, nullptr))
// ... 106 lines not shown
```

### medicalsemseg_amd/csrc/k3pp.h

```cpp
#pragma once
#include "common.h"

struct K3ppParams {
    const void* x;
    long long ldx;
    const void* wp;
    const float* bias;
    void* y;
    long long ldy;
    int N, D, H, W, K, M;
    float* stats;
    float* stats_ws;
    unsigned int* counter;
    const void* nb_y; long long nb_ldy;
    const void* nb_a; long long nb_lda;
    const float* nb_stats;
    float nb_slope, nb_eps; long long nb_S;
    float* nb_dgamma; float* nb_dbeta; int nb_acc;
    int accumulate;
};

bool msseg_k3pp_eligible(const K3ppParams& p);
int msseg_k3pp_launch(const K3ppParams& p, hipStream_t stream);

bool msseg_k3c48_shape_ok(int N, int D, int H, int W, int M);
bool msseg_k3c48_eligible(const K3ppParams& p);
int msseg_k3c48_launch(const K3ppParams& p, hipStream_t stream);

struct K3FinParams {
    const float* ws;
    int R, N, coutb, M;
    float* stats;
    const float* nb_stats;
    float nb_eps; long long nb_S;
    float* nb_dgamma; float* nb_dbeta; int nb_acc;
};
int msseg_k3_stats_finalize(const K3FinParams& f, int ncb, hipStream_t stream);

struct K3WgParams {
    const void* pten; long long ldp;
    const void* qten; long long ldq;
    float* slabs;
    int N, D, H, W, M, K, kblks;
    int dbg_noload;
};
bool msseg_k3wg_pp_eligible(const K3WgParams& p);
int msseg_k3wg_pp_grid(const K3WgParams& p);
int msseg_k3wg_pp_launch(const K3WgParams& p, int gx, hipStream_t stream);

struct StemParams {
    const void* x; long long ldx;
    const void* wp;
    const float* bias;
    void* y; long long ldy;
    int N, D, H, W, M;
    float* stats; float* stats_ws;
    int taps;
    const float* nstats; const float* gamma; const float* beta; float eps, slope;
};
struct StemWgParams {
    const void* x; long long ldx;
    const void* dy; long long lddy;
    float* slabs;
    int N, D, H, W, M;
};
bool msseg_stem_eligible(int dtype, int Cin, int Cout, int k, int s, int pd, long long ldx, long long ldy, const void* y);
int msseg_stem_fwd_launch(const StemParams& p, hipStream_t stream);
int msseg_stem_wgrad_grid(const StemWgParams& p);
int msseg_stem_wgrad_launch(const StemWgParams& p, int gx, hipStream_t stream);

bool msseg_deconv2_fast_eligible(int dtype, int Cin, int Cout, const void* coarse, long long ldc, const void* fine,
                                 long long ldf, const float* bias);
int msseg_deconv2_fwd_launch(const void* x, long long ldx, const void* wp, const float* bias, void* y, long long ldy, int N,
                             int D, int H, int W, int Cin, int Cout, hipStream_t stream);
int msseg_deconv2_bwd_launch(const void* dy, long long lddy, const void* wp, void* dx, long long lddx, int N, int D, int H,
                             int W, int Cin, int Cout, const void* yraw, long long ldyraw, const void* act, long long ldact,
                             const float* fwd_stats, float slope, float eps, float* red, float* dgamma, float* dbeta,
                             int accumulate, float* dbias, int dbias_accumulate, void* scratch, size_t scratch_bytes,
                             hipStream_t stream);

bool msseg_deconv2g_fwd_eligible(int dtype, int Cin, int Cout, const void* coarse, long long ldc, const void* fine,
                                 long long ldf, const float* bias);
int msseg_deconv2g_fwd_launch(const void* x, long long ldx, const void* wp, const float* bias, void* y, long long ldy, int N,
                              int D, int H, int W, int Cin, int Cout, hipStream_t stream);
bool msseg_deconv2g_bwd_eligible(int dtype, int Cin, int Cout, const void* coarse, long long ldc, const void* fine,
                                 long long ldf);
int msseg_deconv2g_bwd_launch(const void* dy, long long lddy, const void* wp, void* dx, long long lddx, float* part, int N,
                              int D, int H, int W, int Cin, int Cout, hipStream_t stream);
bool msseg_linear_regw_eligible(int dtype, long long NV, int Cin, int Cout, const void* x, long long ldx, const void* y,
                                long long ldy, const float* bias);
int msseg_linear_regw_launch(const void* x, long long ldx, const void* wp, const float* bias, void* y, long long ldy,
// ... 2 lines not shown
```

### medicalsemseg_amd/csrc/stem_conv.hip

```cpp
#include "k3pp.h"

namespace {

constexpr int TD = 4, TH = 4, TW = 16;
constexpr int PD = TD + 2, PH = TH + 2, PW = TW + 2;
constexpr int HV = PD * PH * PW;

typedef __attribute__((address_space(3))) unsigned char lds_u8;
typedef __attribute__((ext_vector_type(16))) float f32x16_t;

struct TileCo { int n, d0, h0, w0; };

struct Sched {
    int tiles_w, tiles_h, tiles_d, t_first, t_step, n_my;
    MSSEG_DEVFN void init(int N, int D, int H, int W) {
        tiles_w = (W + TW - 1) / TW; tiles_h = (H + TH - 1) / TH; tiles_d = (D + TD - 1) / TD;
        const int ntiles = N * tiles_d * tiles_h * tiles_w;
        int t_end;
        if ((gridDim.x & 7) == 0) {
            const int chunk = (ntiles + 7) >> 3, xcd = blockIdx.x & 7;
            t_first = xcd * chunk + (blockIdx.x >> 3);
            t_step = gridDim.x >> 3;
            t_end = min(ntiles, (xcd + 1) * chunk);
        } else {
// ... 314 lines not shown

}

bool msseg_stem_eligible(int dtype, int Cin, int Cout, int k, int s, int pd, long long ldx, long long ldy, const void* y) {
    static const bool off = getenv("MSSEG_NO_STEM") != nullptr;
    return !off && dtype == MSSEG_BF16 && Cin == 1 && ((k == 3 && pd == 1) || (k == 1 && pd == 0)) && s == 1 &&
           (Cout % 32 == 0 || Cout % 48 == 0) && Cout <= 256 &&
           ldx >= 1 && (ldy % 4) == 0 && (((uintptr_t)y) & 7) == 0;
}

int msseg_stem_fwd_launch(const StemParams& p, hipStream_t stream) {
    const int cbw = (p.M % 32 == 0) ? 32 : 48;
    const int ncb = p.M / cbw;
    const int tiles = p.N * ceil_div(p.D, TD) * ceil_div(p.H, TH) * ceil_div(p.W, TW);
    int gx = msseg_num_cus() * 2 / ncb;
    gx &= ~7;
    if (gx < 8) gx = 8;
    if (gx > tiles) gx = tiles;
    if (p.nstats != nullptr && p.stats != nullptr) MSSEG_FAIL(MSSEG_EINVAL, "stem_fwd: the normalised form emits no statistics");
    if (p.y == nullptr && p.stats == nullptr) MSSEG_FAIL(MSSEG_EINVAL, "stem_fwd: nothing to produce");
    if (cbw == 32) {
        if (p.nstats) hipLaunchKernelGGL((stem_fwd_kernel<0, 2, 1>), dim3(gx, ncb), dim3(F_THREADS), 0, stream, p);
        else if (p.stats) hipLaunchKernelGGL((stem_fwd_kernel<1, 2>), dim3(gx, ncb), dim3(F_THREADS), 0, stream, p);
        else hipLaunchKernelGGL((stem_fwd_kernel<0, 2>), dim3(gx, ncb), dim3(F_THREADS), 0, stream, p);
    } else {
        if (p.nstats) hipLaunchKernelGGL((stem_fwd_kernel<0, 3, 1>), dim3(gx, ncb), dim3(F_THREADS), 0, stream, p);
        else if (p.stats) hipLaunchKernelGGL((stem_fwd_kernel<1, 3>), dim3(gx, ncb), dim3(F_THREADS), 0, stream, p);
        else hipLaunchKernelGGL((stem_fwd_kernel<0, 3>), dim3(gx, ncb), dim3(F_THREADS), 0, stream, p);
    }
    MSSEG_CHECK_LAUNCH("stem_fwd");
    if (p.stats) {
        K3FinParams f{};
        f.ws = p.stats_ws; f.R = gx; f.N = p.N; f.coutb = cbw; f.M = p.M; f.stats = p.stats;
        return msseg_k3_stats_finalize(f, ncb, stream);
    }
    return MSSEG_OK;
}

int msseg_stem_wgrad_grid(const StemWgParams& p) {
    const int tiles = p.N * ceil_div(p.D, TD) * ceil_div(p.H, TH) * ceil_div(p.W, TW);
    int gx = msseg_num_cus() * 2 / ceil_div(p.M, 32);
    gx &= ~7;
    if (gx < 8) gx = 8;
    if (gx > tiles) gx = tiles;
    return gx;
}

int msseg_stem_wgrad_launch(const StemWgParams& p, int gx, hipStream_t stream) {
    const int lds = 2 * (P_BYTES + 3 * XS_ELEMS * 2 + 64);
    static msseg_lds_attr_once attr;
    if (!attr.ensure((const void*)stem_wgrad_kernel, lds)) MSSEG_FAIL(MSSEG_ELAUNCH, "stem_wgrad: cannot set dynamic LDS size %d", lds);
    hipLaunchKernelGGL(stem_wgrad_kernel, dim3(gx, ceil_div(p.M, 32)), dim3(W_THREADS), lds, stream, p);
    MSSEG_CHECK_LAUNCH("stem_wgrad");
    return MSSEG_OK;
}
```

### medicalsemseg_amd/hip.py

```python
from __future__ import annotations

import ctypes as C
import os
from typing import Optional

import torch

_HERE = os.path.dirname(os.path.abspath(__file__))
LIB_PATH = os.environ.get("MSSEG_LIB") or os.path.join(_HERE, "libmsseg_hip.so")

F32, BF16 = 0, 1
_DT = {torch.float32: F32, torch.bfloat16: BF16}
_LAB = {torch.float32: 0, torch.bfloat16: 1, torch.uint8: 2, torch.int64: 3}

_lib = None

_vp, _ll, _i, _f, _sz = C.c_void_p, C.c_longlong, C.c_int, C.c_float, C.c_size_t

SIGNATURES = {
    "msseg_abi_version": ([], _i),
    "msseg_last_error": ([], C.c_char_p),
    "msseg_num_cus": ([], _i),
    "msseg_packed_weight_bytes": ([_i, _i, _i, _i, _i], _sz),
    "msseg_pack_weights": ([_vp, _vp, _i, _i, _i, _i, _i, _i, _ll, _ll, _ll, _ll, _ll, _i, _i, _vp], _i),
# ... 98 lines not shown
    "msseg_sw_normalize": ([_vp, _vp, _i, _ll, _vp], _i),
    "msseg_sw_gather": ([_vp, _vp, _i, _i, _i, _i, _i, _i, _i, _i, _i, _i, _i, _f, _vp], _i),
    "msseg_box_copy": ([_vp, _ll, _i, _i, _i, _vp, _ll, _i, _i, _i, _i, _i, _i, _vp], _i),
    "msseg_merge_gather_fwd": ([_vp, _ll, _i, _i, _i, _vp, _ll, _i, _i, C.c_uint, _i, _vp], _i),
    "msseg_merge_gather_bwd": ([_vp, _ll, _vp, _ll, _i, _i, _i, _i, _i, C.c_uint, _i, _vp], _i),
    "msseg_argmax_u8": ([_vp, _i, _ll, _vp, _vp], _i),
    "msseg_resample_nearest_u8": ([_vp, _i, _i, _i, _vp, _i, _i, _i, _vp], _i),
    "msseg_majority_vote_u8": ([_vp, _i, _ll, _i, _vp, _vp], _i),
    "msseg_aug_crop_batch": ([_vp, _vp, _i, _i, _i, _i, _vp, _i, _vp, _i, _vp, _i, _vp], _i),
    "msseg_intensity_prep": ([_vp, _i, _i, _i, _i, _i, _i, _f, _f, _i, _f, _f, _vp, _vp, _vp], _i),
    "msseg_resample_spacing": ([_vp, _i, _i, _i, _i, _i, _vp, _i, _i, _i, C.c_double, C.c_double, C.c_double, _vp], _i),
    "msseg_crop_pad_copy": ([_vp, _i, _i, _i, _i, _i, _vp, _vp, _i, _i, _i, _vp, _f, _i, _vp], _i),
    "msseg_slab_counts": ([_vp, _vp, _i, _i, _i, _f, _vp, _vp], _i),
    "msseg_pick_voxels": ([_vp, _i, _vp, _i, _i, _f, _vp, _vp], _i),
    "msseg_aug_crop_multi": ([_vp, _i, _vp, _vp, _i, _i, _vp, _i, _vp, _i, _vp], _i),
    "msseg_sw_gather_batch": ([_vp, _ll, _vp, _ll, _i, _vp, _i, _i, _i, _i, _i, _i, _i, _i, _f, _vp], _i),
    "msseg_sw_blend_batch": ([_vp, _ll, _i, _vp, _vp, _ll, _vp, _ll, _vp, _i, _i, _i, _i, _i, _i, _i, _i, _vp], _i),
    "msseg_deconv_k2s2_bwd_partials_ok": ([_i, _i, _i], _i),
    "msseg_deconv_k2s2_bwd_partials": ([_vp, _ll, _vp, _vp, _sz, _i, _i, _i, _i, _i, _i, _i, _vp], _i),
    "msseg_conv3d_k3_small_ok": ([_i, _i, _i, _i, _i, _i, _i], _i),
    "msseg_conv3d_k3_small_workspace_bytes": ([_i, _i, _i, _i, _i, _i], _sz),
    "msseg_conv3d_k3_small_stage_groups": ([_i, _i, _i, _i, _i, _i], _i),
    "msseg_conv3d_k3_small_partials": ([_vp, _ll, _vp, _vp, _sz, _i, _i, _i, _i, _i, _i, _vp], _i),
    "msseg_conv3d_k3_small_fwd_finish": ([_vp, _i, _vp, _vp, _vp, _f, _f, _vp, _ll, _vp, _ll, _vp, _ll, _vp, _i, _i, _i, _i,
                                          _i, _vp], _i),
    "msseg_conv3d_k3_small_fwd_finish_res": ([_vp, _i, _vp, _vp, _vp, _f, _f, _vp, _ll, _vp, _ll, _vp, _ll, _vp, _ll, _vp, _i, _i, _i, _i,
                                              _i, _vp], _i),
    "msseg_conv3d_k3_small_bwd_finish": ([_vp, _i, _vp, _ll, _vp, _ll, _vp, _vp, _vp, _f, _f, _vp, _vp, _i, _i, _i, _i, _i,
                                          _i, _vp], _i),
    "msseg_avgpool3d_k3": ([_vp, _ll, _vp, _ll, _i, _i, _i, _i, _i, _i, _vp], _i),
    "msseg_hd_edges": ([_vp, _vp, _i, _i, _i, _i, _vp, _vp, _vp, _vp], _i),
    "msseg_hd_directed_workspace_bytes": ([_i, _i, _i], _sz),
    "msseg_hd_directed_hist": ([_vp, _vp, _i, _i, _i, _i, _vp, _vp, _sz, _vp, _i, _vp], _i),
    "msseg_ktimer_enable": ([_i], _i),
    "msseg_ktimer_reset": ([], _i),
    "msseg_ktimer_count": ([], _i),
    "msseg_ktimer_get": ([_i, C.c_char_p, _i, C.POINTER(C.c_float)], _i),
}


def load_library(path: Optional[str] = None):
    global _lib
    if _lib is not None and path is None:
        return _lib
    p = path or LIB_PATH
    if not os.path.exists(p):
        raise RuntimeError(
            f"{p} not found: build it with `python -c 'import __graft_entry__ as g; g.build()'` "
            f"(or `make -C medicalsemseg_amd/csrc`).  There is no CPU fallback.")
    lib = C.CDLL(p)
    for name, (args, res) in SIGNATURES.items():
        fn = getattr(lib, name)
        fn.argtypes = args
        fn.restype = res
    if lib.msseg_abi_version() != 1:
        raise RuntimeError("libmsseg_hip.so ABI version mismatch")
    _lib = lib
    return lib


def lib():
    real = _lib if _lib is not None else load_library()
    if TIMER.enabled:
        return _TimedLib(real)
    return real

# ... 220 lines not shown
    torch.cuda.synchronize()
    out = {}
    buf = C.create_string_buffer(96)
    ms = C.c_float()
    for i in range(L.msseg_ktimer_count()):
        if L.msseg_ktimer_get(i, buf, 96, C.byref(ms)) == 0:
            r = out.setdefault(buf.value.decode(), {"launches": 0, "total_ms": 0.0})
            r["launches"] += 1
            r["total_ms"] += float(ms.value)
    for r in out.values():
        r["avg_ms"] = r["total_ms"] / r["launches"]
    if reset:
        L.msseg_ktimer_reset()
    return out


TIMER = KernelTimer()


_scratch_cache = {}


def scratch(device) -> torch.Tensor:
    key = device.index if device.index is not None else torch.cuda.current_device()
    buf = _scratch_cache.get(key)
    if buf is None:
        buf = torch.zeros(lib().msseg_reduce_scratch_bytes() + 256, dtype=torch.uint8, device=device)
        off = (-buf.data_ptr()) % 256
        buf = buf[off:off + lib().msseg_reduce_scratch_bytes()]
        _scratch_cache[key] = buf
    return buf


def conv3d_k3(x, wp, bias, y, cin, cout, stats=None):
    _need_gpu(x, wp, y)
    N, D, H, W = x.shape[:4]
    nv = N * D * H * W
    esz = x.element_size()
    sc = scratch(x.device) if stats is not None else None

    def go():
        _ck(lib().msseg_conv3d_k3_fwd(_p(x), ld(x), _p(wp), _p(bias), _p(y), ld(y), N, D, H, W, cin, cout, _p(stats),
                                      _p(sc), sc.numel() if sc is not None else 0, dt(x), _stream()), "conv3d_k3_fwd")
    key = "conv3d_k3_fwd"
    if TIMER.enabled:
        key += "/v%d" % lib().msseg_conv3d_k3_kernel(N, D, H, W, cin, cout, dt(x))
    TIMER.launch(key, 2.0 * nv * 27 * cin * cout, nv * (cin + cout) * esz + 27 * cin * cout * esz, go)
    return y


def conv3d_k3_accumulate(x, wp, y, cin, cout, stats):
    _need_gpu(x, wp, y, stats)
    N, D, H, W = x.shape[:4]
    nv = N * D * H * W
    sc = scratch(x.device)
    TIMER.launch("conv3d_k3_fwd/v%d" % (4 if cin == 48 else 3), 2.0 * nv * 27 * cin * cout, nv * (cin + 2 * cout) * x.element_size() + 27 * cin * cout * 2,
                 lambda: _ck(lib().msseg_conv3d_k3_fwd_accumulate(_p(x), ld(x), _p(wp), _p(y), ld(y), N, D, H, W, cin, cout,
                                                                 _p(stats), _p(sc), sc.numel(), dt(x), _stream()),
                             "conv3d_k3_fwd_accumulate"))
    return y


def conv3d_k3_dgrad_inbwd(dy, wp, da, cin, cout, yraw, act, fwd_stats, slope, eps, dgamma=None, dbeta=None,
                          accumulate=False):
    _need_gpu(dy, wp, da, yraw, act, fwd_stats)
    N, D, H, W = dy.shape[:4]
    nv = N * D * H * W
    esz = dy.element_size()
    red = torch.empty(N, cout, 2, dtype=torch.float32, device=dy.device)
    sc = scratch(dy.device)

    def go():
        _ck(lib().msseg_conv3d_k3_dgrad_inbwd(_p(dy), ld(dy), _p(wp), _p(da), ld(da), N, D, H, W, cin, cout, _p(yraw),
                                              ld(yraw), _p(act), ld(act), _p(fwd_stats), slope, eps, _p(red),
                                              _p(dgamma), _p(dbeta), int(accumulate), _p(sc), sc.numel(), dt(dy),
                                              _stream()), "conv3d_k3_dgrad_inbwd")
    key = "conv3d_k3_fwd"
    if TIMER.enabled:
        key += "/v%d" % lib().msseg_conv3d_k3_kernel(N, D, H, W, cin, cout, dt(dy))
    TIMER.launch(key, 2.0 * nv * 27 * cin * cout, nv * (cin + 3 * cout) * esz + 27 * cin * cout * esz, go)
    return red


def conv3d_k3_small_ok(x, cin, cout) -> bool:
    if os.environ.get("MSSEG_NO_K3_SMALL") or x.dim() != 5 or x.dtype != torch.bfloat16:
        return False
    N, D, H, W = x.shape[:4]
    return bool(lib().msseg_conv3d_k3_small_ok(N, D, H, W, cin, cout, BF16))


_k3s_ws = {}


def _k3s_workspace(nbytes, device):
    key = device.index if device.index is not None else torch.cuda.current_device()
    buf = _k3s_ws.get(key)
    if buf is None or buf.numel() * 4 < nbytes:
        if buf is not None:
            _ws_retired.append(buf)
        buf = torch.empty(max(nbytes, 32 << 20) // 4, dtype=torch.float32, device=device)
        _k3s_ws[key] = buf
    return buf


def conv3d_k3_small_partials(x, wp, cin, cout):
# ... 132 lines not shown
    _need_gpu(dy, wp, dx)
    N, D, H, W = dx.shape[:4]
    red = None
    yraw = act = stats = None
    slope = eps = 0.0
    if next_norm is not None:
        yraw, act, stats, slope, eps = next_norm
        red = torch.empty(N, cin, 2, dtype=torch.float32, device=dy.device)
    sc = scratch(dy.device)
    _ck(lib().msseg_deconv_k2s2_bwd_fused(_p(dy), ld(dy), _p(wp), _p(dx), ld(dx), N, D, H, W, cin, cout, _p(yraw),
                                          ld(yraw) if yraw is not None else 0, _p(act), ld(act) if act is not None else 0,
                                          _p(stats), slope, eps, _p(red), _p(dgamma), _p(dbeta), int(accumulate), _p(dbias),
                                          int(dbias_accumulate), _p(sc), sc.numel(), dt(dy), _stream()),
        "deconv_k2s2_bwd_fused")
    return red


def conv3d_gather(x, wp, bias, y, cin, cout, k, s, p):
    _need_gpu(x, wp, y)
    N, D, H, W = x.shape[:4]
    _ck(lib().msseg_conv3d_gather_fwd(_p(x), ld(x), _p(wp), _p(bias), _p(y), ld(y), N, D, H, W, cin, cout, k, s, p,
                                      dt(x), _stream()), "conv3d_gather_fwd")
    return y


def conv3d_stem_norm(x, wp, bias, stats, gamma, beta, eps, slope, y, cout):
    _need_gpu(x, wp, y, stats)
    N, D, H, W = x.shape[:4]
    _ck(lib().msseg_conv3d_stem_norm_fwd(_p(x), ld(x), _p(wp), _p(bias), _p(stats), _p(gamma), _p(beta), eps, slope, _p(y), ld(y),
                                         N, D, H, W, cout, dt(x), _stream()), "conv3d_stem_norm_fwd")
    return y


def conv3d_stem(x, wp, bias, y, cout, stats=None, k=3):
    _need_gpu(x, wp)
    N, D, H, W = x.shape[:4]
    sc = scratch(x.device) if stats is not None else None
    fn = lib().msseg_conv3d_stem_fwd if k == 3 else lib().msseg_conv3d_stem_k1_fwd
    _ck(fn(_p(x), ld(x), _p(wp), _p(bias), _p(y), ld(y) if y is not None else 0, N, D, H, W, cout, _p(stats), _p(sc),
                                    sc.numel() if sc is not None else 0, dt(x), _stream()), "conv3d_stem_fwd")
    return y


def deconv_k2s2(x, wp, bias, y, cin, cout):
    _need_gpu(x, wp, y)
    N, D, H, W = x.shape[:4]
    _ck(lib().msseg_deconv_k2s2_fwd(_p(x), ld(x), _p(wp), _p(bias), _p(y), ld(y), N, D, H, W, cin, cout, dt(x),
                                    _stream()), "deconv_k2s2_fwd")
    return y


def deconv_k2s2_bwd_data(dy, wp, dx, cin, cout):
    _need_gpu(dy, wp, dx)
    N, D, H, W = dx.shape[:4]
    _ck(lib().msseg_deconv_k2s2_bwd_data(_p(dy), ld(dy), _p(wp), _p(dx), ld(dx), N, D, H, W, cin, cout, dt(dy),
                                         _stream()), "deconv_k2s2_bwd_data")
    return dx


def deconv_k4s4(x, wp, bias, y, cin, cout):
    _need_gpu(x, wp, y)
    N, D, H, W = x.shape[:4]
    if tuple(y.shape) != (N, 4 * D, 4 * H, 4 * W, cout):
        raise ValueError(f"deconv_k4s4: output shape {tuple(y.shape)} for input {tuple(x.shape)}, cout {cout}")
    nv = N * D * H * W
    esz = x.element_size()
    TIMER.launch("deconv_k4s4_fwd", 2.0 * nv * 64 * cin * cout, nv * (cin + 64 * cout) * esz + 64 * cin * cout * esz,
                 lambda: _ck(lib().msseg_deconv_k4s4_fwd(_p(x), ld(x), _p(wp), _p(bias), _p(y), ld(y), N, D, H, W, cin, cout,
                                                         dt(x), _stream()), "deconv_k4s4_fwd"))
    return y
# ... 162 lines not shown
def kv_attention_bwd(q, kv, o, lse, dout, heads, scale):
    _need_gpu(q, kv, o, lse, dout)
    B, N, C = q.shape
    M = kv.shape[1]
    dq, dkv = torch.empty_like(q), torch.empty_like(kv)
    nb = lib().msseg_kv_attention_bwd_workspace_bytes(B, N, M, heads, C // heads)
    ws = torch.empty(nb, dtype=torch.uint8, device=q.device)
    _ck(lib().msseg_kv_attention_bwd(_p(q), _p(kv), _p(o), _p(lse), _p(dout), _p(dq), _p(dkv), B, N, M, heads, C // heads,
                                     scale, _p(ws), nb, dt(q), _stream()), "kv_attention_bwd")
    return dq, dkv


def scale_channels(x, scale, y):
    _need_gpu(x, scale, y)
    N, C = x.shape[0], x.shape[-1]
    _ck(lib().msseg_scale_channels(_p(x), _p(scale), _p(y), N, x.numel() // (N * C), C, dt(x), _stream()), "scale_channels")
    return y


def channel_stats(x, stats=None):
    _need_gpu(x)
    N, S, Cc = _nsc(x)
    if stats is None:
        stats = torch.empty(N, Cc, 2, dtype=torch.float32, device=x.device)
    sc = scratch(x.device)
    _ck(lib().msseg_channel_stats(_p(x), ld(x), _p(stats), N, S, Cc, _p(sc), sc.numel(), dt(x), _stream()),
        "channel_stats")
    return stats


def instnorm_act_fwd(x, stats, gamma, beta, y, slope, eps=1e-5, residual=None):
    _need_gpu(x, stats, y)
    N, S, Cc = _nsc(x)
    TIMER.launch("instnorm_act_fwd", 0.0, _nbytes(x, y, residual), lambda: _ck(lib().msseg_instnorm_act_fwd(_p(x), ld(x), _p(stats), _p(gamma), _p(beta), _p(residual),
                                     ld(residual) if residual is not None else 0, _p(y), ld(y), N, S, Cc, eps, slope,
                                     dt(x), _stream()), "instnorm_act_fwd"))
    return y


def instnorm_pool_ok(x, y, pooled) -> bool:
    epc = 16 // x.element_size()
    return (x.dim() == 5 and all(int(d) % 2 == 0 for d in x.shape[1:4]) and x.shape[-1] % epc == 0
            and all(ld(t) % epc == 0 and t.data_ptr() % 16 == 0 for t in (x, y, pooled)))


def instnorm_act_pool_fwd(x, stats, gamma, beta, y, pooled, slope, eps=1e-5):
    _need_gpu(x, stats, y, pooled)
    N, D, H, W, Cc = x.shape
    TIMER.launch("instnorm_act_pool_fwd", 0.0, _nbytes(x, y, pooled), lambda: _ck(lib().msseg_instnorm_act_pool_fwd(_p(x), ld(x), _p(stats), _p(gamma), _p(beta), _p(y), ld(y), _p(pooled), ld(pooled),
                                          N, D, H, W, Cc, eps, slope, dt(x), _stream()), "instnorm_act_pool_fwd"))
    return y, pooled


def instnorm_act_poolbwd_reduce(x, stats, gamma, beta, skip, g, da, slope, eps=1e-5, dgamma=None, dbeta=None,
                                accumulate=False):
    _need_gpu(x, stats, skip, g, da)
    N, D, H, W, Cc = x.shape
    red = torch.empty(N, Cc, 2, dtype=torch.float32, device=x.device)
    sc = scratch(x.device)
    TIMER.launch("instnorm_act_poolbwd_reduce", 0.0, _nbytes(x, skip, g, da), lambda: _ck(lib().msseg_instnorm_act_poolbwd_reduce(_p(x), ld(x), _p(stats), _p(gamma), _p(beta), _p(skip), ld(skip), _p(g),
                                                ld(g), _p(da), ld(da), _p(red), _p(dgamma), _p(dbeta), int(accumulate),
                                                N, D, H, W, Cc, eps, slope, _p(sc), sc.numel(), dt(x), _stream()),
        "instnorm_act_poolbwd_reduce"))
    return red


def instnorm_act_bwd(x, stats, gamma, y, dy, dx, slope, eps=1e-5, dres=None, dgamma=None, dbeta=None,
                     accumulate=False, beta=None):
    _need_gpu(x, stats, dy, dx)
    red = instnorm_act_bwd_reduce(x, stats, gamma, y, dy, slope, eps, dgamma, dbeta, accumulate, beta)
    instnorm_act_bwd_apply(x, stats, gamma, y, dy, red, dx, slope, eps, dres, beta)
    return red


def instnorm_act_bwd_reduce(x, stats, gamma, y, dy, slope, eps=1e-5, dgamma=None, dbeta=None, accumulate=False, beta=None):
    _need_gpu(x, stats, dy)
    N, S, Cc = _nsc(x)
    red = torch.empty(N, Cc, 2, dtype=torch.float32, device=x.device)
    sc = scratch(x.device)
    TIMER.launch("instnorm_act_bwd_reduce", 0.0, _nbytes(x, y, dy), lambda: _ck(lib().msseg_instnorm_act_bwd_reduce(_p(x), ld(x), _p(stats), _p(gamma), _p(beta), _p(y),
                                            ld(y) if y is not None else 0, _p(dy), ld(dy), _p(red),
                                            _p(dgamma), _p(dbeta), int(accumulate), N, S, Cc, eps, slope, _p(sc),
                                            sc.numel(), dt(x), _stream()), "instnorm_act_bwd_reduce"))
    return red


def instnorm_act_bwd_apply(x, stats, gamma, y, dy, red, dx, slope, eps=1e-5, dres=None, beta=None):
    _need_gpu(x, stats, dy, dx, red)
    N, S, Cc = _nsc(x)
    TIMER.launch("instnorm_act_bwd_apply", 0.0, _nbytes(x, y, dy, dx, dres), lambda: _ck(lib().msseg_instnorm_act_bwd_apply(_p(x), ld(x), _p(stats), _p(gamma), _p(beta), _p(y),
                                           ld(y) if y is not None else 0, _p(dy), ld(dy), _p(red),
                                           _p(dx), ld(dx), _p(dres), ld(dres) if dres is not None else 0, N, S, Cc, eps,
                                           slope, dt(x), _stream()), "instnorm_act_bwd_apply"))
    return red


def maxpool2_fwd(x, y):
    _need_gpu(x, y)
    N, D, H, W, Cc = x.shape
    _ck(lib().msseg_maxpool2_fwd(_p(x), ld(x), _p(y), ld(y), N, D, H, W, Cc, dt(x), _stream()), "maxpool2_fwd")
    return y


def maxpool2_bwd(x, dy, dx, accumulate=False):
    _need_gpu(x, dy, dx)
    N, D, H, W, Cc = x.shape
    _ck(lib().msseg_maxpool2_bwd(_p(x), ld(x), _p(dy), ld(dy), _p(dx), ld(dx), N, D, H, W, Cc, int(accumulate), dt(x),
                                 _stream()), "maxpool2_bwd")
    return dx


def to_channels_last(src: torch.Tensor, dst: torch.Tensor):
    _need_gpu(src, dst)
    src = src.contiguous()
    N, Cc = src.shape[0], src.shape[1]
    S = src.numel() // (N * Cc)
    _ck(lib().msseg_ncdhw_to_ndhwc(_p(src), dt(src), _p(dst), ld(dst), dt(dst), N, Cc, S, _stream()), "ncdhw_to_ndhwc")
    return dst


def to_channels_first(src: torch.Tensor, dst: torch.Tensor):
    _need_gpu(src, dst)
    N, Cc = dst.shape[0], dst.shape[1]
    S = dst.numel() // (N * Cc)
    assert dst.is_contiguous()
    _ck(lib().msseg_ndhwc_to_ncdhw(_p(src), ld(src), dt(src), _p(dst), dt(dst), N, Cc, S, _stream()), "ndhwc_to_ncdhw")
# ... 491 lines not shown
```

### medicalsemseg_amd/layers.py

```python
from __future__ import annotations

import os

from typing import Optional

import torch

from . import hip

weights_epoch = 0


def bump_weights_epoch():
    global weights_epoch
    weights_epoch += 1


class _PackRegistry:

    def __init__(self):
        self.groups = {}

    def add(self, device, dtype, src, dst, job):
        g = self.groups.setdefault((device, dtype), {"jobs": [], "table": None, "keep": []})
# ... 158 lines not shown
    owner = getattr(p, "_msseg_gowner", None)
    if owner is not None and not getattr(p, "_msseg_kgrad", False):
        p._msseg_kgrad = True
        p._msseg_gepoch = owner._gepoch
        return p.grad, True
    if owner is not None and getattr(p, "_msseg_gepoch", -1) != owner._gepoch:
        p._msseg_gepoch = owner._gepoch
        return p.grad, False
    return p.grad, True


def _empty_like_vol(x, C, dtype=None):
    return torch.empty(x.shape[:-1] + (C,), dtype=dtype or x.dtype, device=x.device)


def _norm_grad_bufs(nrm):
    if nrm.gamma is not None and nrm.gamma.requires_grad:
        dg, acc = _grad_buf(nrm.gamma)
        db, _ = _grad_buf(nrm.beta)
        return dg, db, acc
    return None, None, False


class Conv3:

    def __init__(self, weight: torch.nn.Parameter, bias: Optional[torch.nn.Parameter]):
        self.w, self.b = weight, bias
        self.cout, self.cin = weight.shape[0], weight.shape[1]
        self.cache = PackedCache()

    def _gather(self, dtype):
        return self.cin % (8 if dtype == torch.bfloat16 else 4) != 0

    def fwd(self, x, out=None, want_stats=False):
        dtype = x.dtype
        if want_stats and out is None and self.halves_ok(tuple(x.shape[:4]), dtype):
            return self.fwd_halves(x)
        y = out if out is not None else _empty_like_vol(x, self.cout)
        stats = None
        if self._gather(dtype):
            wp = self.cache.get(self.w, dtype, "g", lambda: hip.pack_conv_gather(self.w.detach(), dtype))
            if (self.cin == 1 and dtype == torch.bfloat16 and (self.cout % 32 == 0 or self.cout % 48 == 0) and self.cout <= 256
                    and not os.environ.get("MSSEG_NO_STEM")):
                if want_stats and x.shape[0] <= 8:
                    stats = torch.empty(x.shape[0], self.cout, 2, dtype=torch.float32, device=x.device)
                hip.conv3d_stem(x, wp, self.b, y, self.cout, stats)
            else:
                hip.conv3d_gather(x, wp, self.b, y, self.cin, self.cout, 3, 1, 1)
        else:
            vol = tuple(x.shape[:4])
            wp = self.cache.get(self.w, dtype, ("f", vol), lambda: hip.pack_conv_k3(self.w.detach(), dtype, vol=vol))
            if want_stats and x.shape[0] <= 8:
                stats = torch.empty(x.shape[0], self.cout, 2, dtype=torch.float32, device=x.device)
            hip.conv3d_k3(x, wp, self.b, y, self.cin, self.cout, stats)
        if want_stats:
            return y, (stats if stats is not None else hip.channel_stats(y))
        return y

    def halves_ok(self, vol, dtype) -> int:
        if dtype != torch.bfloat16 or os.environ.get("MSSEG_NO_SPLIT_CAT"):
            return 0
        if self.cin == 96 and hip.lib().msseg_conv3d_k3_kernel(*vol, 48, self.cout, hip.BF16) == 4:
            return 48
        if (INFERENCE_FORWARD and self.cin in (64, 128) and self.cout % 32 == 0 and not os.environ.get("MSSEG_NO_KSPLIT_INFER")
                and hip.lib().msseg_conv3d_k3_kernel(*vol, 32, self.cout, hip.BF16) == 3):
            return 32
        return 0

    def fwd_halves(self, x):
        dtype, vol = x.dtype, tuple(x.shape[:4])
        h = self.halves_ok(vol, dtype)
        y = _empty_like_vol(x, self.cout)
        stats = torch.empty(x.shape[0], self.cout, 2, dtype=torch.float32, device=x.device)
        for i in range(self.cin // h):
            wi = self.w.detach()[:, i * h:(i + 1) * h]
            pi = self.cache.get(wi, dtype, ("fp", i, h, vol), lambda wi=wi: hip.pack_conv_k3(wi, dtype, vol=vol))
            xi = x[..., i * h:(i + 1) * h]
            if i == 0:
                hip.conv3d_k3(xi, pi, self.b, y, h, self.cout)
            else:
                hip.conv3d_k3_accumulate(xi, pi, y, h, self.cout, stats)
        return y, stats

    def split_ok(self, vol, dtype, ca, cb_) -> bool:
        if (os.environ.get("MSSEG_NO_SPLIT_CAT") or dtype != torch.bfloat16 or ca + cb_ != self.cin or ca != 32 or cb_ != 32
                or self.cout % 32 or vol[0] > 8):
            return False
        return hip.lib().msseg_conv3d_k3_kernel(*vol, 32, self.cout, hip.BF16) == 3

    def fwd_split(self, xa, xb):
        dtype = xa.dtype
        vol = tuple(xa.shape[:4])
        wa, wb = self.w.detach()[:, :32], self.w.detach()[:, 32:]
        pa = self.cache.get(wa, dtype, ("fa", vol), lambda: hip.pack_conv_k3(wa, dtype, vol=vol))
        pb = self.cache.get(wb, dtype, ("fb", vol), lambda: hip.pack_conv_k3(wb, dtype, vol=vol))
        y = _empty_like_vol(xa, self.cout)
        hip.conv3d_k3(xa, pa, self.b, y, 32, self.cout)
        stats = torch.empty(xa.shape[0], self.cout, 2, dtype=torch.float32, device=xa.device)
        hip.conv3d_k3_accumulate(xb, pb, y, 32, self.cout, stats)
        return y, stats

    def dgrad_accumulate_ok(self, dy) -> bool:
        if dy.dtype != torch.bfloat16 or self.cout not in (32, 48) or dy.shape[0] > 4 or os.environ.get("MSSEG_NO_DGRAD_ACCUM"):
            return False
        vol = tuple(dy.shape[:4])
        return hip.lib().msseg_conv3d_k3_kernel(*vol, self.cout, self.cin, hip.BF16) == (4 if self.cout == 48 else 3)

    def bwd(self, x, dy, need_dx=True, dx_out=None, bias_grad_is_zero=False, next_norm=None, accumulate_dx=False):
        dtype = x.dtype
        if self.w.requires_grad:
            g, acc = _grad_buf(self.w)
            if self._gather(dtype):
                WGRAD_SIDE.run(lambda: hip.conv3d_gather_wgrad(x, dy, g, self.cin, self.cout, 3, 1, 1, acc), x, dy)
            else:
                WGRAD_SIDE.run(lambda: hip.conv3d_k3_wgrad(x, dy, g, self.cin, self.cout, acc), x, dy)
        if self.b is not None and self.b.requires_grad:
            g, acc = _grad_buf(self.b)
            if bias_grad_is_zero:
                if not acc and not getattr(self.b, "_msseg_grad_is_zero", False):
                    g.zero_()
                    self.b._msseg_grad_is_zero = getattr(self.b, "_msseg_gowner", None) is not None
            else:
                hip.channel_sum(dy, g, acc)
        if not need_dx:
            return None
        if self._gather(dtype):
            raise NotImplementedError("input gradient of a few-channel stem conv is never needed on this path")
        vol = tuple(dy.shape[:4])
        if accumulate_dx:
            assert dx_out is not None and next_norm is None and self.dgrad_accumulate_ok(dy)
            wp = self.cache.get(self.w, dtype, ("d", vol),
                                lambda: hip.pack_conv_k3(self.w.detach(), dtype, dgrad=True, vol=vol))
            unused = torch.empty(dy.shape[0], self.cin, 2, dtype=torch.float32, device=dy.device)
            hip.conv3d_k3_accumulate(dy, wp, dx_out, self.cout, self.cin, unused)
            return dx_out
        if hip.conv3d_k3_small_ok(dy, self.cout, self.cin):
            wp = self.cache.get(self.w, dtype, "ds", lambda: hip.pack_conv_k3(self.w.detach(), dtype, dgrad=True, cb=32))
            part, ng = hip.conv3d_k3_small_partials(dy, wp, self.cout, self.cin)
            dx = dx_out if dx_out is not None else _empty_like_vol(dy, self.cin)
            if next_norm is not None:
                nrm, yraw, stats, act = next_norm
                dg, db, acc = _norm_grad_bufs(nrm)
                hip.conv3d_k3_small_bwd_finish(part, ng, dx, (yraw, stats, nrm.gamma, nrm.beta, nrm.eps, nrm.slope),
                                               dg, db, acc)
                return dx, APPLIED
            return hip.conv3d_k3_small_bwd_finish(part, ng, dx)
        wp = self.cache.get(self.w, dtype, ("d", vol),
                            lambda: hip.pack_conv_k3(self.w.detach(), dtype, dgrad=True, vol=vol))
        dx = dx_out if dx_out is not None else _empty_like_vol(dy, self.cin)
        if next_norm is not None:
            nrm, yraw, stats, act = next_norm
            if dy.shape[0] <= 8 and self.cin % 4 == 0:
                dg = db = None
                acc = False
                if nrm.gamma is not None and nrm.gamma.requires_grad:
                    dg, acc = _grad_buf(nrm.gamma)
                    db, _ = _grad_buf(nrm.beta)
                red = hip.conv3d_k3_dgrad_inbwd(dy, wp, dx, self.cout, self.cin, yraw, act, stats, nrm.slope, nrm.eps,
                                                dg, db, acc)
                return dx, red
            hip.conv3d_k3(dy, wp, None, dx, self.cout, self.cin)
            return dx, None
        hip.conv3d_k3(dy, wp, None, dx, self.cout, self.cin)
        return dx


class Conv1:

    def __init__(self, weight, bias):
        self.w, self.b = weight, bias
        self.cout, self.cin = weight.shape[0], weight.shape[1]
        self.cache = PackedCache()

    def _gather(self, dtype):
        return self.cin % (8 if dtype == torch.bfloat16 else 4) != 0

    def fwd(self, x, out=None, want_stats=False):
        dtype = x.dtype
        y = out if out is not None else _empty_like_vol(x, self.cout)
        if self._gather(dtype):
            wp = self.cache.get(self.w, dtype, "g", lambda: hip.pack_conv_gather(self.w.detach(), dtype))
            if (want_stats and self.cin == 1 and dtype == torch.bfloat16 and x.dim() == 5 and x.shape[0] <= 8 and hip.ld(y) == self.cout
                    and (self.cout % 32 == 0 or self.cout % 48 == 0) and self.cout <= 256 and not os.environ.get("MSSEG_NO_STEM")):
                stats = torch.empty(x.shape[0], self.cout, 2, dtype=torch.float32, device=x.device)
                hip.conv3d_stem(x, wp, self.b, y, self.cout, stats, k=1)
                return y, stats
            hip.conv3d_gather(x, wp, self.b, y, self.cin, self.cout, 1, 1, 0)
        elif (self.cout <= 4 and self.cin <= 64 and x.shape[-1] == self.cin and self.w.is_contiguous()
              and not os.environ.get("MSSEG_NO_HEAD_KERNEL")):
            hip.conv3d_k1_head(x, self.w.detach(), self.b, y, self.cin, self.cout)
        else:
            wp = self.cache.get(self.w, dtype, "f",
# ... 197 lines not shown
        if self.gamma is not None and self.gamma.requires_grad:
            dg, acc = _grad_buf(self.gamma)
            db, acc2 = _grad_buf(self.beta)
            assert acc == acc2
        hip.instnorm_act_bwd(y_raw, stats, self.gamma, a_in, da, dy, self.slope, self.eps, dres, dg, db, acc, self.beta)
        return (dy, dres) if want_dres else dy


class ConvNormAct:

    def __init__(self, conv: Conv3, norm: InstNormAct):
        self.conv, self.norm = conv, norm

    def fwd(self, x, out=None, pooled=None):
        cv, nm = self.conv, self.norm
        if (INFERENCE_FORWARD and pooled is None and cv.cin == 1 and x.dtype == torch.bfloat16 and x.shape[0] <= 8
                and (cv.cout % 32 == 0 or cv.cout % 48 == 0) and cv.cout <= 256 and not os.environ.get("MSSEG_NO_STEM")
                and not os.environ.get("MSSEG_NO_STEM_TWICE")):
            wp = cv.cache.get(cv.w, x.dtype, "g", lambda: hip.pack_conv_gather(cv.w.detach(), x.dtype))
            stats = torch.empty(x.shape[0], cv.cout, 2, dtype=torch.float32, device=x.device)
            hip.conv3d_stem(x, wp, cv.b, None, cv.cout, stats)
            a = out if out is not None else _empty_like_vol(x, cv.cout)
            hip.conv3d_stem_norm(x, wp, cv.b, stats, nm.gamma, nm.beta, nm.eps, nm.slope, a, cv.cout)
            return a, (x, None, stats, a)
        if (not cv._gather(x.dtype) and hip.conv3d_k3_small_ok(x, cv.cin, cv.cout)
                and (pooled is None or hip.instnorm_pool_ok(x, x, pooled))):
            wp = cv.cache.get(cv.w, x.dtype, "fs", lambda: hip.pack_conv_k3(cv.w.detach(), x.dtype, cb=32))
            part, ng = hip.conv3d_k3_small_partials(x, wp, cv.cin, cv.cout)
            y = _empty_like_vol(x, cv.cout)
            a = out if out is not None else _empty_like_vol(x, cv.cout)
            stats = torch.empty(x.shape[0], cv.cout, 2, dtype=torch.float32, device=x.device)
            hip.conv3d_k3_small_fwd_finish(part, ng, cv.b, nm.gamma, nm.beta, nm.eps, nm.slope, y, a, pooled, stats)
            return a, (x, y, stats, a)
        y, stats = self.conv.fwd(x, want_stats=True)
        a, stats = self.norm.fwd(y, out, stats=stats, pooled=pooled)
        return a, (x, y, stats, a)

    def bwd(self, saved, da, need_dx=True, red=None, next_saved=None, next_cna=None):
        x, y, stats, a = saved
        dy = self.norm.bwd(y, stats, a, da, red=red)
        if next_cna is not None and need_dx:
            nx, ny, nstats, na = next_saved
            return self.conv.bwd(x, dy, True, bias_grad_is_zero=True, next_norm=(next_cna.norm, ny, nstats, na))
        return self.conv.bwd(x, dy, need_dx, bias_grad_is_zero=True)


def maxpool_fwd(x):
    N, D, H, W, C = x.shape
    y = torch.empty(N, D // 2, H // 2, W // 2, C, dtype=x.dtype, device=x.device)
    return hip.maxpool2_fwd(x, y)


class ResBlock:

    def __init__(self, conv1_w, conv2_w, conv3_w=None, slope=0.01):
        self.c1, self.c2 = Conv3(conv1_w, None), Conv3(conv2_w, None)
        self.c3 = Conv1(conv3_w, None) if conv3_w is not None else None
        self.n1, self.n2 = InstNormAct(None, None, slope), InstNormAct(None, None, slope)
        self.n3 = InstNormAct(None, None, 1.0) if conv3_w is not None else None

    @staticmethod
    def _small_unit(conv, nrm, x, residual=None, out=None):
        wp = conv.cache.get(conv.w, x.dtype, "fs", lambda: hip.pack_conv_k3(conv.w.detach(), x.dtype, cb=32))
        part, ng = hip.conv3d_k3_small_partials(x, wp, conv.cin, conv.cout)
        y = _empty_like_vol(x, conv.cout)
        a = out if out is not None else _empty_like_vol(x, conv.cout)
        stats = torch.empty(x.shape[0], conv.cout, 2, dtype=torch.float32, device=x.device)
        hip.conv3d_k3_small_fwd_finish(part, ng, conv.b, nrm.gamma, nrm.beta, nrm.eps, nrm.slope, y, a, None, stats, residual)
        return a, y, stats

    def fwd(self, x, out=None):
        small = (not self.c1._gather(x.dtype) and hip.conv3d_k3_small_ok(x, self.c1.cin, self.c1.cout)
                 and hip.conv3d_k3_small_ok(x, self.c2.cin, self.c2.cout))
        if small:
            a1, y1, s1 = self._small_unit(self.c1, self.n1, x)
        else:
# ... 160 lines not shown
```

Before: 532.7 vol/s.

## Defer conv stats finalize into the consuming instnorm kernels

Conv3d k3, stem and dgrad-in-bwd kernels can now skip their separate stats/red finalize launch and pass a descriptor on instead. The following instnorm forward, norm+pool forward and bwd-apply kernels then reduce the per-block partial workspace into LDS at their start. This removes one small kernel launch and a global round trip per conv+norm pair. In exchange, every block of the consumer redoes the finalize reduction, and there is extra LDS use and host-side descriptor plumbing.

New measurement: 526.4 vol/s. 1.2% lower.

```diff
diff --git a/include/msseg.h b/include/msseg.h
--- a/include/msseg.h
+++ b/include/msseg.h
@@ -58,6 +58,26 @@
                                 long long ldact, const float* fwd_stats, float slope, float eps, float* red,
                                 float* dgamma, float* dbeta, int accumulate, void* scratch, size_t scratch_bytes,
                                 int dtype, msseg_stream_t stream);
+typedef struct msseg_fin_desc {
+    const float* ws;
+    float* out;
+    const float* nb_stats;
+    float* nb_dgamma;
+    float* nb_dbeta;
+    long long nb_S;
+    float nb_eps;
+    int nb_acc;
+    int R, N, coutb, ncb, M;
+    int mode;
+} msseg_fin_desc;
+int msseg_conv3d_k3_fwd_deferred(const void* x, long long ldx, const void* wp, const float* bias, void* y, long long ldy,
+                                 int N, int D, int H, int W, int Cin, int Cout, float* stats, void* scratch,
+                                 size_t scratch_bytes, int dtype, msseg_fin_desc* desc, msseg_stream_t stream);
+int msseg_conv3d_k3_dgrad_inbwd_deferred(const void* dy, long long lddy, const void* wp, void* da, long long ldda, int N,
+                                         int D, int H, int W, int Cin, int Cout, const void* yraw, long long ldyraw,
+                                         const void* act, long long ldact, const float* fwd_stats, float slope, float eps,
+                                         float* red, float* dgamma, float* dbeta, int accumulate, void* scratch,
+                                         size_t scratch_bytes, int dtype, msseg_fin_desc* desc, msseg_stream_t stream);
 int msseg_conv3d_k3s2_fwd(const void* x, long long ldx, const void* wp, const float* bias, void* y, long long ldy,
                           int N, int ID, int IH, int IW, int Cin, int Cout, int dtype, msseg_stream_t stream);
 int msseg_zero_stuff2(const void* dy, long long lddy, void* out, long long ldo, int N, int OD, int OH, int OW, int ID,
@@ -65,6 +85,9 @@
 int msseg_conv3d_stem_fwd(const void* x, long long ldx, const void* wp, const float* bias, void* y, long long ldy,
                           int N, int D, int H, int W, int Cout, float* stats, void* scratch, size_t scratch_bytes,
                           int dtype, msseg_stream_t stream);
+int msseg_conv3d_stem_fwd_deferred(const void* x, long long ldx, const void* wp, const float* bias, void* y, long long ldy,
+                                   int N, int D, int H, int W, int Cout, float* stats, void* scratch, size_t scratch_bytes,
+                                   int dtype, msseg_fin_desc* desc, msseg_stream_t stream);
 int msseg_conv3d_stem_k1_fwd(const void* x, long long ldx, const void* wp, const float* bias, void* y, long long ldy,
                              int N, int D, int H, int W, int Cout, float* stats, void* scratch, size_t scratch_bytes,
                              int dtype, msseg_stream_t stream);
@@ -205,6 +228,19 @@
                                  const float* beta, const void* y, long long ldy, const void* dy, long long lddy, const float* red, void* dx,
                                  long long lddx, void* dres, long long lddres, int N, long long S, int C, float eps,
                                  float slope, int dtype, msseg_stream_t stream);
+int msseg_instnorm_act_fwd_deferred(const void* x, long long ldx, const float* stats, const float* gamma,
+                                    const float* beta, const void* residual, long long ldr, void* y, long long ldy, int N,
+                                    long long S, int C, float eps, float slope, int dtype, const msseg_fin_desc* desc,
+                                    msseg_stream_t stream);
+int msseg_instnorm_act_pool_fwd_deferred(const void* x, long long ldx, const float* stats, const float* gamma,
+                                         const float* beta, void* y, long long ldy, void* pooled, long long ldp, int N,
+                                         int D, int H, int W, int C, float eps, float slope, int dtype,
+                                         const msseg_fin_desc* desc, msseg_stream_t stream);
+int msseg_instnorm_act_bwd_apply_deferred(const void* x, long long ldx, const float* stats, const float* gamma,
+                                          const float* beta, const void* y, long long ldy, const void* dy, long long lddy,
+                                          const float* red, void* dx, long long lddx, void* dres, long long lddres, int N,
+                                          long long S, int C, float eps, float slope, int dtype,
+                                          const msseg_fin_desc* desc, msseg_stream_t stream);
 int msseg_maxpool2_fwd(const void* x, long long ldx, void* y, long long ldy, int N, int D, int H, int W, int C,
                        int dtype, msseg_stream_t stream);
 int msseg_maxpool2_bwd(const void* x, long long ldx, const void* dy, long long lddy, void* dx, long long lddx,
diff --git a/medicalsemseg_amd/csrc/conv3d_k3_c48.hip b/medicalsemseg_amd/csrc/conv3d_k3_c48.hip
--- a/medicalsemseg_amd/csrc/conv3d_k3_c48.hip
+++ b/medicalsemseg_amd/csrc/conv3d_k3_c48.hip
@@ -369,7 +369,7 @@
         f.ws = p.stats_ws; f.R = gx; f.N = p.N; f.coutb = 16; f.M = p.M; f.stats = p.stats;
         f.nb_stats = (STATS == 2) ? p.nb_stats : nullptr; f.nb_eps = p.nb_eps; f.nb_S = p.nb_S;
         f.nb_dgamma = p.nb_dgamma; f.nb_dbeta = p.nb_dbeta; f.nb_acc = p.nb_acc;
-        return msseg_k3_stats_finalize(f, ncb, stream);
+        return msseg_k3_stats_finish(f, ncb, p.defer, stream);
     }
     return MSSEG_OK;
 }
diff --git a/medicalsemseg_amd/csrc/conv3d_k3_pp.hip b/medicalsemseg_amd/csrc/conv3d_k3_pp.hip
--- a/medicalsemseg_amd/csrc/conv3d_k3_pp.hip
+++ b/medicalsemseg_amd/csrc/conv3d_k3_pp.hip
@@ -353,7 +353,7 @@
         f.ws = p.stats_ws; f.R = gx; f.N = p.N; f.coutb = 32; f.M = p.M; f.stats = p.stats;
         f.nb_stats = (STATS == 2) ? p.nb_stats : nullptr; f.nb_eps = p.nb_eps; f.nb_S = p.nb_S;
         f.nb_dgamma = p.nb_dgamma; f.nb_dbeta = p.nb_dbeta; f.nb_acc = p.nb_acc;
-        return msseg_k3_stats_finalize(f, ncb, stream);
+        return msseg_k3_stats_finish(f, ncb, p.defer, stream);
     }
     return MSSEG_OK;
 }
diff --git a/medicalsemseg_amd/csrc/elementwise.hip b/medicalsemseg_amd/csrc/elementwise.hip
--- a/medicalsemseg_amd/csrc/elementwise.hip
+++ b/medicalsemseg_amd/csrc/elementwise.hip
@@ -1,4 +1,5 @@
 #include "common.h"
+#include "k3pp.h"
 
 #include <stdarg.h>
 #include <string.h>
@@ -347,7 +348,36 @@
     long long S; int C; float eps, slope;
     long long rows_per_block; int groups, rows_par;
     float* ws; unsigned int* counter; float* dgamma; float* dbeta; int accumulate;
+    K3FinParams fin; int fin_ncb;
 };
+
+constexpr int NORM_FIN_MAX = 1024;
+MSSEG_DEVFN void norm_fin_fwd(const K3FinParams& f, int ncb, int n, float* fin, float* dst, bool write) {
+    const int Ls = f.coutb * 2;
+    for (int cb = 0; cb < ncb; ++cb) {
+        const float* tot = k3_fin_fwd_rows(f, cb, n, fin);
+        for (int i = threadIdx.x; i < Ls; i += 256) {
+            const int c = cb * f.coutb + (i >> 1), k = i & 1;
+            if (c < f.M) {
+                dst[c * 2 + k] = tot[i];
+                if (write) f.stats[((long long)n * f.M + c) * 2 + k] = tot[i];
+            }
+        }
+    }
+}
+MSSEG_DEVFN void norm_fin_bwd(const K3FinParams& f, int ncb, int n, float* fin, float* dst, bool write) {
+    for (int cb = 0; cb < ncb; ++cb) {
+        const float* tot = k3_fin_bwd_rows(f, cb, fin);
+        const int cl = threadIdx.x, cg = cb * f.coutb + cl;
+        if (cl < f.coutb && cg < f.M) {
+            float a, b2;
+            k3_fin_bwd_value(f, tot, cl, cg, n, a, b2);
+            dst[cg * 2 + 0] = a;
+            dst[cg * 2 + 1] = b2;
+            if (write) k3_fin_bwd_write(f, tot, cl, cg);
+        }
+    }
+}
 
 MSSEG_DEVFN void mean_rstd(const float* stats, int n, int C, int c, long long S, float eps, float& mean, float& rstd) {
     const float inv = 1.0f / (float)S;
@@ -358,12 +388,29 @@
     rstd = rsqrtf(var + eps);
 }
 
-template <typename T, bool VEC, int MODE>
+template <typename T, bool VEC, int MODE, bool FIN = false>
 __global__ __launch_bounds__(MODE == 1 ? RED_THREADS : 256) void instnorm_kernel(const NormParams p) {
     constexpr int W = VEC ? DT<T>::EPC : 1;
     __shared__ float red[(MODE == 1) ? RED_THREADS * 2 * W : 1];
     __shared__ int lflag;
+    __shared__ __attribute__((aligned(16))) float fin[FIN ? K3_FIN_LDS_FLOATS : 4];
+    __shared__ float fval[FIN ? NORM_FIN_MAX : 1];
     const int n = blockIdx.y;
+    const float* st_src = p.stats;
+    const float* red_src = p.red;
+    constexpr int sn_fixed = FIN && MODE == 0, rn_fixed = FIN && MODE == 2;
+    if constexpr (FIN) {
+        static_assert(MODE != 1, "the reduce pass consumes no deferred finalize");
+        if constexpr (MODE == 0) {
+            norm_fin_fwd(p.fin, p.fin_ncb, n, fin, fval, blockIdx.x == 0);
+            st_src = fval;
+        } else {
+            norm_fin_bwd(p.fin, p.fin_ncb, n, fin, fval, blockIdx.x == 0 && n == 0);
+            red_src = fval;
+        }
+        __syncthreads();
+    }
+    const int sn = sn_fixed ? 0 : n, rn = rn_fixed ? 0 : n;
     const int g = threadIdx.x % p.groups, rl = threadIdx.x / p.groups;
     const long long r0 = (long long)blockIdx.x * p.rows_per_block;
     long long r1 = r0 + p.rows_per_block;
@@ -384,14 +431,14 @@
 #pragma unroll
         for (int e = 0; e < W; ++e) {
             const int c = act ? gg * W + e : 0;
-            mean_rstd(p.stats, n, p.C, c, p.S, p.eps, mean[e], rstd[e]);
+            mean_rstd(st_src, sn, p.C, c, p.S, p.eps, mean[e], rstd[e]);
             const float ga = p.gamma ? p.gamma[c] : 1.f;
             sc[e] = rstd[e] * ga;
             sh[e] = (p.beta ? p.beta[c] : 0.f) - mean[e] * sc[e];
             a0[e] = a1[e] = 0.f;
             if constexpr (MODE == 2) {
-                k0[e] = p.red[((long long)n * p.C + c) * 2 + 0] * invS;
-                k1[e] = p.red[((long long)n * p.C + c) * 2 + 1] * invS;
+                k0[e] = red_src[((long long)rn * p.C + c) * 2 + 0] * invS;
+                k1[e] = red_src[((long long)rn * p.C + c) * 2 + 1] * invS;
             }
         }
         if (act && rl < p.rows_par) {
@@ -513,11 +560,20 @@
     void* y; long long ldy;
     void* pooled; long long ldp;
     int N, D, H, W, C; float eps, slope;
+    K3FinParams fin; int fin_ncb;
 };
 
-template <typename T>
+template <typename T, bool FIN = false>
 __global__ __launch_bounds__(256) void instnorm_pool_fwd_kernel(const NormPoolParams p) {
     constexpr int WD = DT<T>::EPC;
+    __shared__ __attribute__((aligned(16))) float fin[FIN ? K3_FIN_LDS_FLOATS : 4];
+    __shared__ float fval[FIN ? NORM_FIN_MAX : 1];
+    const float* st_src = p.stats;
+    if constexpr (FIN) {
+        for (int nn = 0; nn < p.N; ++nn) norm_fin_fwd(p.fin, p.fin_ncb, nn, fin, fval + nn * p.C * 2, blockIdx.x == 0);
+        st_src = fval;
+        __syncthreads();
+    }
     const int OD = p.D / 2, OH = p.H / 2, OW = p.W / 2;
     const unsigned ug = (unsigned)(p.C / WD);
     const unsigned total = (unsigned)((long long)p.N * OD * OH * OW * ug);
@@ -536,7 +592,7 @@
         for (int e = 0; e < WD; ++e) {
             const int c = g * WD + e;
             float mean, rstd;
-            mean_rstd(p.stats, n, p.C, c, S, p.eps, mean, rstd);
+            mean_rstd(st_src, n, p.C, c, S, p.eps, mean, rstd);
             sc[e] = rstd * (p.gamma ? p.gamma[c] : 1.f);
             sh[e] = (p.beta ? p.beta[c] : 0.f) - mean * sc[e];
             best[e] = -INFINITY;
@@ -817,6 +873,16 @@
     p.rows_per_block = ceil_div_ll(p.S, blocks);
     blocks = ceil_div_ll(p.S, p.rows_per_block);
     dim3 grid((unsigned)blocks, N);
+    if constexpr (MODE != 1) {
+        if (p.fin.ws != nullptr) {
+            if (vec && p.C * 2 <= NORM_FIN_MAX) {
+                hipLaunchKernelGGL((instnorm_kernel<T, true, MODE, true>), grid, dim3(NTHR), 0, st, p);
+                MSSEG_CHECK_LAUNCH("instnorm");
+                return MSSEG_OK;
+            }
+            if (int rc = msseg_k3_stats_finalize(p.fin, p.fin_ncb, st)) return rc;
+        }
+    }
     if (vec) hipLaunchKernelGGL((instnorm_kernel<T, true, MODE>), grid, dim3(NTHR), 0, st, p);
     else hipLaunchKernelGGL((instnorm_kernel<T, false, MODE>), grid, dim3(NTHR), 0, st, p);
     MSSEG_CHECK_LAUNCH("instnorm");
@@ -1338,11 +1404,33 @@
                return launch_stats<bf16_t>(x, ldx, out, 1, rows, C, 1, accumulate, scratch, (hipStream_t)stream));
 }
 
+static int fin_desc_check(const msseg_fin_desc* desc, int mode, const float* out, int N, int C, const char* who, bool* deferred) {
+    *deferred = desc != nullptr && desc->ws != nullptr;
+    if (!*deferred) return MSSEG_OK;
+    if (desc->mode != mode || desc->out != out || desc->N != N || desc->M != C || desc->R < 1 || desc->ncb < 1 ||
+        desc->coutb < 1 || desc->ncb * desc->coutb < C || desc->N * desc->coutb * 2 > K3_FIN_LDS_FLOATS - 256 * 4 ||
+        (mode == 1 && desc->nb_stats == nullptr))
+        MSSEG_FAIL(MSSEG_EINVAL, "%s: the deferred-finalize descriptor does not describe this call's %s", who,
+                   mode ? "red" : "stats");
+    return MSSEG_OK;
+}
+
 int msseg_instnorm_act_fwd(const void* x, long long ldx, const float* stats, const float* gamma, const float* beta,
                            const void* residual, long long ldr, void* y, long long ldy, int N, long long S, int C,
                            float eps, float slope, int dtype, msseg_stream_t stream) {
+    return msseg_instnorm_act_fwd_deferred(x, ldx, stats, gamma, beta, residual, ldr, y, ldy, N, S, C, eps, slope, dtype,
+                                           nullptr, stream);
+}
+
+int msseg_instnorm_act_fwd_deferred(const void* x, long long ldx, const float* stats, const float* gamma,
+                                    const float* beta, const void* residual, long long ldr, void* y, long long ldy, int N,
+                                    long long S, int C, float eps, float slope, int dtype, const msseg_fin_desc* desc,
+                                    msseg_stream_t stream) {
     if (!x || !stats || !y || N < 1 || S < 1 || C < 1) MSSEG_FAIL(MSSEG_EINVAL, "instnorm_act_fwd: bad args");
     NormParams p{};
+    bool deferred;
+    if (int rc = fin_desc_check(desc, 0, stats, N, C, "instnorm_act_fwd", &deferred)) return rc;
+    if (deferred) { p.fin = msseg_fin_params(*desc); p.fin_ncb = desc->ncb; }
     p.x = x; p.ldx = ldx; p.stats = stats; p.gamma = gamma; p.beta = beta; p.res = residual; p.ldr = ldr;
     p.y = y; p.ldy = ldy; p.S = S; p.C = C; p.eps = eps; p.slope = slope;
     const int esz = dtype == MSSEG_F32 ? 4 : 2;
@@ -1452,6 +1540,14 @@
 int msseg_instnorm_act_pool_fwd(const void* x, long long ldx, const float* stats, const float* gamma, const float* beta,
                                 void* y, long long ldy, void* pooled, long long ldp, int N, int D, int H, int W, int C,
                                 float eps, float slope, int dtype, msseg_stream_t stream) {
+    return msseg_instnorm_act_pool_fwd_deferred(x, ldx, stats, gamma, beta, y, ldy, pooled, ldp, N, D, H, W, C, eps, slope,
+                                                dtype, nullptr, stream);
+}
+
+int msseg_instnorm_act_pool_fwd_deferred(const void* x, long long ldx, const float* stats, const float* gamma,
+                                         const float* beta, void* y, long long ldy, void* pooled, long long ldp, int N,
+                                         int D, int H, int W, int C, float eps, float slope, int dtype,
+                                         const msseg_fin_desc* desc, msseg_stream_t stream) {
     if (!x || !stats || !y || !pooled || N < 1 || D < 2 || H < 2 || W < 2 || C < 1)
         MSSEG_FAIL(MSSEG_EINVAL, "instnorm_act_pool_fwd: bad args");
     if ((D | H | W) & 1) MSSEG_FAIL(MSSEG_EINVAL, "instnorm_act_pool_fwd: odd spatial size %dx%dx%d", D, H, W);
@@ -1461,10 +1557,23 @@
         MSSEG_FAIL(MSSEG_EINVAL, "instnorm_act_pool_fwd: needs 16-byte aligned rows and a channel count multiple of %d", 16 / esz);
     const long long total = (long long)N * (D / 2) * (H / 2) * (W / 2) * (C / (16 / esz));
     if (total >= 0x7fffffffLL) MSSEG_FAIL(MSSEG_EINVAL, "instnorm_act_pool_fwd: too many elements");
-    NormPoolParams p{x, ldx, stats, gamma, beta, y, ldy, pooled, ldp, N, D, H, W, C, eps, slope};
+    NormPoolParams p{x, ldx, stats, gamma, beta, y, ldy, pooled, ldp, N, D, H, W, C, eps, slope, K3FinParams{}, 0};
     const int g = grid_for(total, 1);
-    DISPATCH_T(dtype, hipLaunchKernelGGL(instnorm_pool_fwd_kernel<float>, dim3(g), dim3(256), 0, (hipStream_t)stream, p),
-               hipLaunchKernelGGL(instnorm_pool_fwd_kernel<bf16_t>, dim3(g), dim3(256), 0, (hipStream_t)stream, p));
+    bool deferred;
+    if (int rc = fin_desc_check(desc, 0, stats, N, C, "instnorm_act_pool_fwd", &deferred)) return rc;
+    if (deferred) {
+        p.fin = msseg_fin_params(*desc); p.fin_ncb = desc->ncb;
+        if ((long long)N * C * 2 <= NORM_FIN_MAX) {
+            DISPATCH_T(dtype,
+                       hipLaunchKernelGGL((instnorm_pool_fwd_kernel<float, true>), dim3(g), dim3(256), 0, (hipStream_t)stream, p),
+                       hipLaunchKernelGGL((instnorm_pool_fwd_kernel<bf16_t, true>), dim3(g), dim3(256), 0, (hipStream_t)stream, p));
+            MSSEG_CHECK_LAUNCH("instnorm_act_pool_fwd");
+            return MSSEG_OK;
+        }
+        if (int rc = msseg_k3_stats_finalize(p.fin, p.fin_ncb, (hipStream_t)stream)) return rc;
+    }
+    DISPATCH_T(dtype, hipLaunchKernelGGL((instnorm_pool_fwd_kernel<float>), dim3(g), dim3(256), 0, (hipStream_t)stream, p),
+               hipLaunchKernelGGL((instnorm_pool_fwd_kernel<bf16_t>), dim3(g), dim3(256), 0, (hipStream_t)stream, p));
     MSSEG_CHECK_LAUNCH("instnorm_act_pool_fwd");
     return MSSEG_OK;
 }
@@ -1525,8 +1634,23 @@
                                  const float* beta, const void* y, long long ldy, const void* dy, long long lddy, const float* red, void* dx,
                                  long long lddx, void* dres, long long lddres, int N, long long S, int C, float eps,
                                  float slope, int dtype, msseg_stream_t stream) {
+    return msseg_instnorm_act_bwd_apply_deferred(x, ldx, stats, gamma, beta, y, ldy, dy, lddy, red, dx, lddx, dres, lddres,
+                                                 N, S, C, eps, slope, dtype, nullptr, stream);
+}
+
+int msseg_instnorm_act_bwd_apply_deferred(const void* x, long long ldx, const float* stats, const float* gamma,
+                                          const float* beta, const void* y, long long ldy, const void* dy, long long lddy,
+                                          const float* red, void* dx, long long lddx, void* dres, long long lddres, int N,
+                                          long long S, int C, float eps, float slope, int dtype,
+                                          const msseg_fin_desc* desc, msseg_stream_t stream) {
     if (!x || !stats || !dy || !red || !dx) MSSEG_FAIL(MSSEG_EINVAL, "instnorm_act_bwd_apply: null pointer");
     NormParams p{};
+    bool deferred;
+    if (int rc = fin_desc_check(desc, 1, red, N, C, "instnorm_act_bwd_apply", &deferred)) return rc;
+    if (deferred) {
+        if (desc->nb_stats != stats) MSSEG_FAIL(MSSEG_EINVAL, "instnorm_act_bwd_apply: the deferred sums belong to other statistics");
+        p.fin = msseg_fin_params(*desc); p.fin_ncb = desc->ncb;
+    }
     p.x = x; p.ldx = ldx; p.stats = stats; p.gamma = gamma; p.beta = beta; p.y = (void*)y; p.ldy = ldy; p.dy = dy; p.lddy = lddy;
     p.red = (float*)red; p.dx = dx; p.lddx = lddx; p.dres = dres; p.lddres = lddres;
     p.S = S; p.C = C; p.eps = eps; p.slope = slope;
diff --git a/medicalsemseg_amd/csrc/igemm_fwd.hip b/medicalsemseg_amd/csrc/igemm_fwd.hip
--- a/medicalsemseg_amd/csrc/igemm_fwd.hip
+++ b/medicalsemseg_amd/csrc/igemm_fwd.hip
@@ -30,6 +30,7 @@
     int cout_block;
     float* stats;
     float* stats_ws;
+    msseg_fin_desc* defer;
     unsigned int* counter;
     const void* nb_y; long long nb_ldy;
     const void* nb_a; long long nb_lda;
@@ -596,43 +597,20 @@
 }
 
 __global__ __launch_bounds__(256) void k3_stats_finalize_kernel(const K3FinParams f) {
-    __shared__ __attribute__((aligned(16))) float fin[256 * 4 + 8 * 48 * 2];
+    __shared__ __attribute__((aligned(16))) float fin[K3_FIN_LDS_FLOATS];
     const int tid = threadIdx.x;
-    const int L = f.N * f.coutb * 2;
     const int cbase = blockIdx.x * f.coutb;
     if (f.nb_stats == nullptr) {
         const int n = blockIdx.y, Ls = f.coutb * 2;
-        block_rows_sum<256>(f.ws + (long long)blockIdx.x * f.R * L + n * Ls, f.R, Ls, fin, L);
-        const float* tot = fin + 256 * 4;
+        const float* tot = k3_fin_fwd_rows(f, blockIdx.x, n, fin);
         for (int i = tid; i < Ls; i += 256) {
             const int cl = i >> 1, k = i & 1;
             if (cbase + cl < f.M) f.stats[((long long)n * f.M + cbase + cl) * 2 + k] = tot[i];
         }
         return;
     }
-    block_rows_sum<256>(f.ws + (long long)blockIdx.x * f.R * L, f.R, L, fin);
-    const float* tot = fin + 256 * 4;
-    if (tid < f.coutb && cbase + tid < f.M) {
-        const int cg = cbase + tid;
-        float g0 = 0.f, g1 = 0.f;
-        const float inv = 1.0f / (float)f.nb_S;
-        for (int nn = 0; nn < f.N; ++nn) {
-            const float a = tot[(nn * f.coutb + tid) * 2], b0 = tot[(nn * f.coutb + tid) * 2 + 1];
-            const float fs = f.nb_stats[((long long)nn * f.M + cg) * 2], fs2 = f.nb_stats[((long long)nn * f.M + cg) * 2 + 1];
-            const float mean = fs * inv;
-            float var = fs2 * inv - mean * mean;
-            var = var > 0.f ? var : 0.f;
-            const float b2 = rsqrtf(var + f.nb_eps) * (b0 - mean * a);
-            g0 += a;
-            g1 += b2;
-            f.stats[((long long)nn * f.M + cg) * 2 + 0] = a;
-            f.stats[((long long)nn * f.M + cg) * 2 + 1] = b2;
-        }
-        if (f.nb_dgamma != nullptr) {
-            f.nb_dbeta[cg] = f.nb_acc ? f.nb_dbeta[cg] + g0 : g0;
-            f.nb_dgamma[cg] = f.nb_acc ? f.nb_dgamma[cg] + g1 : g1;
-        }
-    }
+    const float* tot = k3_fin_bwd_rows(f, blockIdx.x, fin);
+    if (tid < f.coutb && cbase + tid < f.M) k3_fin_bwd_write(f, tot, tid, cbase + tid);
 }
 
 template <typename T, int NTAPS, int SRC, int EPI, int TD, int TH, int TW, int WAVES, int NT, int STRIDE = 1, int NSL = 1, int DIAG = 0>
@@ -669,7 +647,7 @@
         f.ws = p.stats_ws; f.R = gx; f.N = p.N; f.coutb = C::COUTB; f.M = p.M; f.stats = p.stats;
         f.nb_stats = p.nb_y ? p.nb_stats : nullptr; f.nb_eps = p.nb_eps; f.nb_S = p.nb_S;
         f.nb_dgamma = p.nb_dgamma; f.nb_dbeta = p.nb_dbeta; f.nb_acc = p.nb_acc;
-        return msseg_k3_stats_finalize(f, ncb, stream);
+        return msseg_k3_stats_finish(f, ncb, p.defer, stream);
     }
     return MSSEG_OK;
 }
@@ -757,6 +735,16 @@
     return MSSEG_OK;
 }
 
+int msseg_k3_stats_finish(const K3FinParams& f, int ncb, K3FinDesc* defer, hipStream_t stream) {
+    if (defer == nullptr) return msseg_k3_stats_finalize(f, ncb, stream);
+    K3FinDesc d{};
+    d.ws = f.ws; d.out = f.stats; d.nb_stats = f.nb_stats; d.nb_dgamma = f.nb_dgamma; d.nb_dbeta = f.nb_dbeta;
+    d.nb_S = f.nb_S; d.nb_eps = f.nb_eps; d.nb_acc = f.nb_acc;
+    d.R = f.R; d.N = f.N; d.coutb = f.coutb; d.ncb = ncb; d.M = f.M; d.mode = f.nb_stats ? 1 : 0;
+    *defer = d;
+    return MSSEG_OK;
+}
+
 extern "C" int msseg_debug_phase_cycles(unsigned long long* out8) {
     return hipMemcpyFromSymbol(out8, HIP_SYMBOL(g_phase_cycles), 8 * sizeof(unsigned long long)) == hipSuccess ? 0 : -1;
 }
@@ -799,7 +787,7 @@
                        int D, int H, int W, int Cin, int Cout, float* stats, void* scratch, size_t scratch_bytes,
                        const void* nb_y, long long nb_ldy, const void* nb_a, long long nb_lda, const float* nb_stats,
                        float nb_slope, float nb_eps, float* nb_dgamma, float* nb_dbeta, int nb_acc, int dtype,
-                       msseg_stream_t stream);
+                       msseg_stream_t stream, K3FinDesc* defer = nullptr);
 
 int msseg_conv3d_k3_fwd(const void* x, long long ldx, const void* wp, const float* bias, void* y, long long ldy,
                         int N, int D, int H, int W, int Cin, int Cout, float* stats, void* scratch,
@@ -847,11 +835,35 @@
                        act, ldact, fwd_stats, slope, eps, dgamma, dbeta, accumulate, dtype, stream);
 }
 
+int msseg_conv3d_k3_fwd_deferred(const void* x, long long ldx, const void* wp, const float* bias, void* y, long long ldy,
+                                 int N, int D, int H, int W, int Cin, int Cout, float* stats, void* scratch,
+                                 size_t scratch_bytes, int dtype, msseg_fin_desc* desc, msseg_stream_t stream) {
+    if (!stats || !desc) MSSEG_FAIL(MSSEG_EINVAL, "conv3d_k3_fwd_deferred: needs stats and a descriptor");
+    *desc = K3FinDesc{};
+    return k3_fwd_impl(x, ldx, wp, bias, y, ldy, N, D, H, W, Cin, Cout, stats, scratch, scratch_bytes, nullptr, 0, nullptr,
+                       0, nullptr, 0.f, 0.f, nullptr, nullptr, 0, dtype, stream, desc);
+}
+
+int msseg_conv3d_k3_dgrad_inbwd_deferred(const void* dy, long long lddy, const void* wp, void* da, long long ldda, int N,
+                                         int D, int H, int W, int Cin, int Cout, const void* yraw, long long ldyraw,
+                                         const void* act, long long ldact, const float* fwd_stats, float slope, float eps,
+                                         float* red, float* dgamma, float* dbeta, int accumulate, void* scratch,
+                                         size_t scratch_bytes, int dtype, msseg_fin_desc* desc, msseg_stream_t stream) {
+    if (!yraw || !act || !fwd_stats || !red || !desc) MSSEG_FAIL(MSSEG_EINVAL, "conv3d_k3_dgrad_inbwd_deferred: null pointer");
+    if ((dgamma == nullptr) != (dbeta == nullptr)) MSSEG_FAIL(MSSEG_EINVAL, "conv3d_k3_dgrad_inbwd_deferred: dgamma/dbeta go together");
+    const int esz = dtype == MSSEG_F32 ? 4 : 2;
+    if (Cout % 4 || (ldyraw % 4) || (ldact % 4) || ((uintptr_t)yraw % (4 * esz)) || ((uintptr_t)act % (4 * esz)))
+        MSSEG_FAIL(MSSEG_EINVAL, "conv3d_k3_dgrad_inbwd_deferred: channel count / strides must be multiples of 4");
+    *desc = K3FinDesc{};
+    return k3_fwd_impl(dy, lddy, wp, nullptr, da, ldda, N, D, H, W, Cin, Cout, red, scratch, scratch_bytes, yraw, ldyraw,
+                       act, ldact, fwd_stats, slope, eps, dgamma, dbeta, accumulate, dtype, stream, desc);
+}
+
 static int k3_fwd_impl(const void* x, long long ldx, const void* wp, const float* bias, void* y, long long ldy, int N,
                        int D, int H, int W, int Cin, int Cout, float* stats, void* scratch, size_t scratch_bytes,
                        const void* nb_y, long long nb_ldy, const void* nb_a, long long nb_lda, const float* nb_stats,
                        float nb_slope, float nb_eps, float* nb_dgamma, float* nb_dbeta, int nb_acc, int dtype,
-                       msseg_stream_t stream) {
+                       msseg_stream_t stream, K3FinDesc* defer) {
     const int esz = dtype == MSSEG_F32 ? 4 : 2;
     int rc = check_common(x, ldx, wp, y, ldy, dtype, esz);
     if (rc) return rc;
@@ -873,6 +885,7 @@
         p.nb_y = nb_y; p.nb_ldy = nb_ldy; p.nb_a = nb_a; p.nb_lda = nb_lda; p.nb_stats = nb_stats;
         p.nb_slope = nb_slope; p.nb_eps = nb_eps; p.nb_S = (long long)D * H * W;
         p.nb_dgamma = nb_dgamma; p.nb_dbeta = nb_dbeta; p.nb_acc = nb_acc;
+        p.defer = defer;
     }
     if (dtype == MSSEG_BF16) {
         K3ppParams pp{};
@@ -882,6 +895,7 @@
         pp.nb_y = p.nb_y; pp.nb_ldy = p.nb_ldy; pp.nb_a = p.nb_a; pp.nb_lda = p.nb_lda; pp.nb_stats = p.nb_stats;
         pp.nb_slope = p.nb_slope; pp.nb_eps = p.nb_eps; pp.nb_S = p.nb_S;
         pp.nb_dgamma = p.nb_dgamma; pp.nb_dbeta = p.nb_dbeta; pp.nb_acc = p.nb_acc;
+        pp.defer = p.defer;
         if (Cin == 48 && msseg_k3c48_shape_ok(N, D, H, W, Cout)) {
             if (!msseg_k3c48_eligible(pp))
                 MSSEG_FAIL(MSSEG_EINVAL, "conv3d_k3: 48-input-channel layer on a large grid needs 16-byte aligned x, 8-byte "
@@ -968,7 +982,7 @@
 
 static int stem_fwd_taps(const void* x, long long ldx, const void* wp, const float* bias, void* y, long long ldy, int N, int D,
                          int H, int W, int Cout, float* stats, void* scratch, size_t scratch_bytes, int dtype, int taps,
-                         msseg_stream_t stream);
+                         msseg_stream_t stream, K3FinDesc* defer = nullptr);
 
 int msseg_conv3d_stem_fwd(const void* x, long long ldx, const void* wp, const float* bias, void* y, long long ldy,
                           int N, int D, int H, int W, int Cout, float* stats, void* scratch, size_t scratch_bytes,
@@ -976,6 +990,14 @@
     return stem_fwd_taps(x, ldx, wp, bias, y, ldy, N, D, H, W, Cout, stats, scratch, scratch_bytes, dtype, 27, stream);
 }
 
+int msseg_conv3d_stem_fwd_deferred(const void* x, long long ldx, const void* wp, const float* bias, void* y, long long ldy,
+                                   int N, int D, int H, int W, int Cout, float* stats, void* scratch, size_t scratch_bytes,
+                                   int dtype, msseg_fin_desc* desc, msseg_stream_t stream) {
+    if (!stats || !desc) MSSEG_FAIL(MSSEG_EINVAL, "conv3d_stem_fwd_deferred: needs stats and a descriptor");
+    *desc = K3FinDesc{};
+    return stem_fwd_taps(x, ldx, wp, bias, y, ldy, N, D, H, W, Cout, stats, scratch, scratch_bytes, dtype, 27, stream, desc);
+}
+
 int msseg_conv3d_stem_k1_fwd(const void* x, long long ldx, const void* wp, const float* bias, void* y, long long ldy,
                              int N, int D, int H, int W, int Cout, float* stats, void* scratch, size_t scratch_bytes,
                              int dtype, msseg_stream_t stream) {
@@ -984,7 +1006,7 @@
 
 static int stem_fwd_taps(const void* x, long long ldx, const void* wp, const float* bias, void* y, long long ldy, int N, int D,
                          int H, int W, int Cout, float* stats, void* scratch, size_t scratch_bytes, int dtype, int taps,
-                         msseg_stream_t stream) {
+                         msseg_stream_t stream, K3FinDesc* defer) {
     if (!x || !wp || (!y && !stats) || N < 1 || D < 1 || H < 1 || W < 1) MSSEG_FAIL(MSSEG_EINVAL, "conv3d_stem: bad args");
     if (!msseg_stem_eligible(dtype, 1, Cout, 3, 1, 1, ldx, y ? ldy : 4, y))
         MSSEG_FAIL(MSSEG_EINVAL, "conv3d_stem: bf16, Cout a multiple of 32 or 48 (<= 256), 8-byte aligned output rows only");
@@ -997,6 +1019,7 @@
             MSSEG_FAIL(MSSEG_EWORKSPACE, "conv3d_stem: fused statistics need a scratch of %zu bytes", msseg_reduce_scratch_bytes());
         sp.stats = stats;
         sp.stats_ws = (float*)((unsigned char*)scratch + MSSEG_SCRATCH_COUNTER_BYTES);
+        sp.defer = defer;
     }
     return msseg_stem_fwd_launch(sp, (hipStream_t)stream);
 }
diff --git a/medicalsemseg_amd/csrc/k3pp.h b/medicalsemseg_amd/csrc/k3pp.h
--- a/medicalsemseg_amd/csrc/k3pp.h
+++ b/medicalsemseg_amd/csrc/k3pp.h
@@ -18,6 +18,7 @@
     float nb_slope, nb_eps; long long nb_S;
     float* nb_dgamma; float* nb_dbeta; int nb_acc;
     int accumulate;
+    msseg_fin_desc* defer;
 };
 
 bool msseg_k3pp_eligible(const K3ppParams& p);
@@ -36,6 +37,53 @@
     float* nb_dgamma; float* nb_dbeta; int nb_acc;
 };
 int msseg_k3_stats_finalize(const K3FinParams& f, int ncb, hipStream_t stream);
+
+typedef msseg_fin_desc K3FinDesc;
+int msseg_k3_stats_finish(const K3FinParams& f, int ncb, K3FinDesc* defer, hipStream_t stream);
+static inline K3FinParams msseg_fin_params(const K3FinDesc& d) {
+    K3FinParams f{};
+    f.ws = d.ws; f.R = d.R; f.N = d.N; f.coutb = d.coutb; f.M = d.M; f.stats = d.out;
+    f.nb_stats = d.mode == 1 ? d.nb_stats : nullptr; f.nb_eps = d.nb_eps; f.nb_S = d.nb_S;
+    f.nb_dgamma = d.nb_dgamma; f.nb_dbeta = d.nb_dbeta; f.nb_acc = d.nb_acc;
+    return f;
+}
+
+constexpr int K3_FIN_LDS_FLOATS = 256 * 4 + MSSEG_STATS_NMAX * 48 * 2;
+MSSEG_DEVFN const float* k3_fin_fwd_rows(const K3FinParams& f, int cb, int n, float* fin) {
+    const int L = f.N * f.coutb * 2, Ls = f.coutb * 2;
+    block_rows_sum<256>(f.ws + (long long)cb * f.R * L + n * Ls, f.R, Ls, fin, L);
+    return fin + 256 * 4;
+}
+MSSEG_DEVFN const float* k3_fin_bwd_rows(const K3FinParams& f, int cb, float* fin) {
+    const int L = f.N * f.coutb * 2;
+    block_rows_sum<256>(f.ws + (long long)cb * f.R * L, f.R, L, fin);
+    return fin + 256 * 4;
+}
+MSSEG_DEVFN void k3_fin_bwd_value(const K3FinParams& f, const float* tot, int cl, int cg, int nn, float& a, float& b2) {
+    const float inv = 1.0f / (float)f.nb_S;
+    a = tot[(nn * f.coutb + cl) * 2];
+    const float b0 = tot[(nn * f.coutb + cl) * 2 + 1];
+    const float fs = f.nb_stats[((long long)nn * f.M + cg) * 2], fs2 = f.nb_stats[((long long)nn * f.M + cg) * 2 + 1];
+    const float mean = fs * inv;
+    float var = fs2 * inv - mean * mean;
+    var = var > 0.f ? var : 0.f;
+    b2 = rsqrtf(var + f.nb_eps) * (b0 - mean * a);
+}
+MSSEG_DEVFN void k3_fin_bwd_write(const K3FinParams& f, const float* tot, int cl, int cg) {
+    float g0 = 0.f, g1 = 0.f;
+    for (int nn = 0; nn < f.N; ++nn) {
+        float a, b2;
+        k3_fin_bwd_value(f, tot, cl, cg, nn, a, b2);
+        g0 += a;
+        g1 += b2;
+        f.stats[((long long)nn * f.M + cg) * 2 + 0] = a;
+        f.stats[((long long)nn * f.M + cg) * 2 + 1] = b2;
+    }
+    if (f.nb_dgamma != nullptr) {
+        f.nb_dbeta[cg] = f.nb_acc ? f.nb_dbeta[cg] + g0 : g0;
+        f.nb_dgamma[cg] = f.nb_acc ? f.nb_dgamma[cg] + g1 : g1;
+    }
+}
 
 struct K3WgParams {
     const void* pten; long long ldp;
@@ -57,6 +105,7 @@
     float* stats; float* stats_ws;
     int taps;
     const float* nstats; const float* gamma; const float* beta; float eps, slope;
+    msseg_fin_desc* defer;
 };
 struct StemWgParams {
     const void* x; long long ldx;
diff --git a/medicalsemseg_amd/csrc/stem_conv.hip b/medicalsemseg_amd/csrc/stem_conv.hip
--- a/medicalsemseg_amd/csrc/stem_conv.hip
+++ b/medicalsemseg_amd/csrc/stem_conv.hip
@@ -370,7 +370,7 @@
     if (p.stats) {
         K3FinParams f{};
         f.ws = p.stats_ws; f.R = gx; f.N = p.N; f.coutb = cbw; f.M = p.M; f.stats = p.stats;
-        return msseg_k3_stats_finalize(f, ncb, stream);
+        return msseg_k3_stats_finish(f, ncb, p.defer, stream);
     }
     return MSSEG_OK;
 }
diff --git a/medicalsemseg_amd/hip.py b/medicalsemseg_amd/hip.py
--- a/medicalsemseg_amd/hip.py
+++ b/medicalsemseg_amd/hip.py
@@ -154,6 +154,15 @@
     "msseg_hd_edges": ([_vp, _vp, _i, _i, _i, _i, _vp, _vp, _vp, _vp], _i),
     "msseg_hd_directed_workspace_bytes": ([_i, _i, _i], _sz),
     "msseg_hd_directed_hist": ([_vp, _vp, _i, _i, _i, _i, _vp, _vp, _sz, _vp, _i, _vp], _i),
+    "msseg_conv3d_k3_fwd_deferred": ([_vp, _ll, _vp, _vp, _vp, _ll, _i, _i, _i, _i, _i, _i, _vp, _vp, _sz, _i, _vp, _vp], _i),
+    "msseg_conv3d_k3_dgrad_inbwd_deferred": ([_vp, _ll, _vp, _vp, _ll, _i, _i, _i, _i, _i, _i, _vp, _ll, _vp, _ll, _vp, _f, _f,
+                                              _vp, _vp, _vp, _i, _vp, _sz, _i, _vp, _vp], _i),
+    "msseg_conv3d_stem_fwd_deferred": ([_vp, _ll, _vp, _vp, _vp, _ll, _i, _i, _i, _i, _i, _vp, _vp, _sz, _i, _vp, _vp], _i),
+    "msseg_instnorm_act_fwd_deferred": ([_vp, _ll, _vp, _vp, _vp, _vp, _ll, _vp, _ll, _i, _ll, _i, _f, _f, _i, _vp, _vp], _i),
+    "msseg_instnorm_act_pool_fwd_deferred": ([_vp, _ll, _vp, _vp, _vp, _vp, _ll, _vp, _ll, _i, _i, _i, _i, _i, _f, _f, _i,
+                                              _vp, _vp], _i),
+    "msseg_instnorm_act_bwd_apply_deferred": ([_vp, _ll, _vp, _vp, _vp, _vp, _ll, _vp, _ll, _vp, _vp, _ll, _vp, _ll, _i, _ll,
+                                               _i, _f, _f, _i, _vp, _vp], _i),
     "msseg_ktimer_enable": ([_i], _i),
     "msseg_ktimer_reset": ([], _i),
     "msseg_ktimer_count": ([], _i),
@@ -440,14 +449,43 @@
     return buf
 
 
-def conv3d_k3(x, wp, bias, y, cin, cout, stats=None):
+FUSED_FINALIZE = not os.environ.get("MSSEG_NO_FUSED_FINALIZE")
+
+
+class FinDesc(C.Structure):
+    _fields_ = [("ws", _vp), ("out", _vp), ("nb_stats", _vp), ("nb_dgamma", _vp), ("nb_dbeta", _vp), ("nb_S", _ll),
+                ("nb_eps", _f), ("nb_acc", _i), ("R", _i), ("N", _i), ("coutb", _i), ("ncb", _i), ("M", _i), ("mode", _i)]
+
+
+def _defer_on(t: Optional[torch.Tensor], defer: bool):
+    if not (defer and FUSED_FINALIZE and t is not None):
+        return None
+    t._msseg_fin = FinDesc()
+    return t._msseg_fin
+
+
+def _take_fin(t: torch.Tensor):
+    d = getattr(t, "_msseg_fin", None)
+    if d is None:
+        return None, None
+    t._msseg_fin = None
+    return d, C.addressof(d)
+
+
+def conv3d_k3(x, wp, bias, y, cin, cout, stats=None, defer=False):
     _need_gpu(x, wp, y)
     N, D, H, W = x.shape[:4]
     nv = N * D * H * W
     esz = x.element_size()
     sc = scratch(x.device) if stats is not None else None
+    desc = _defer_on(stats, defer)
 
     def go():
+        if desc is not None:
+            _ck(lib().msseg_conv3d_k3_fwd_deferred(_p(x), ld(x), _p(wp), _p(bias), _p(y), ld(y), N, D, H, W, cin, cout,
+                                                   _p(stats), _p(sc), sc.numel(), dt(x), C.addressof(desc), _stream()),
+                "conv3d_k3_fwd_deferred")
+            return
         _ck(lib().msseg_conv3d_k3_fwd(_p(x), ld(x), _p(wp), _p(bias), _p(y), ld(y), N, D, H, W, cin, cout, _p(stats),
                                       _p(sc), sc.numel() if sc is not None else 0, dt(x), _stream()), "conv3d_k3_fwd")
     key = "conv3d_k3_fwd"
@@ -470,15 +508,23 @@
 
 
 def conv3d_k3_dgrad_inbwd(dy, wp, da, cin, cout, yraw, act, fwd_stats, slope, eps, dgamma=None, dbeta=None,
-                          accumulate=False):
+                          accumulate=False, defer=False):
     _need_gpu(dy, wp, da, yraw, act, fwd_stats)
     N, D, H, W = dy.shape[:4]
     nv = N * D * H * W
     esz = dy.element_size()
     red = torch.empty(N, cout, 2, dtype=torch.float32, device=dy.device)
     sc = scratch(dy.device)
+    desc = _defer_on(red, defer)
 
     def go():
+        if desc is not None:
+            _ck(lib().msseg_conv3d_k3_dgrad_inbwd_deferred(_p(dy), ld(dy), _p(wp), _p(da), ld(da), N, D, H, W, cin, cout,
+                                                           _p(yraw), ld(yraw), _p(act), ld(act), _p(fwd_stats), slope, eps,
+                                                           _p(red), _p(dgamma), _p(dbeta), int(accumulate), _p(sc),
+                                                           sc.numel(), dt(dy), C.addressof(desc), _stream()),
+                "conv3d_k3_dgrad_inbwd_deferred")
+            return
         _ck(lib().msseg_conv3d_k3_dgrad_inbwd(_p(dy), ld(dy), _p(wp), _p(da), ld(da), N, D, H, W, cin, cout, _p(yraw),
                                               ld(yraw), _p(act), ld(act), _p(fwd_stats), slope, eps, _p(red),
                                               _p(dgamma), _p(dbeta), int(accumulate), _p(sc), sc.numel(), dt(dy),
@@ -677,10 +723,16 @@
     return y
 
 
-def conv3d_stem(x, wp, bias, y, cout, stats=None, k=3):
+def conv3d_stem(x, wp, bias, y, cout, stats=None, k=3, defer=False):
     _need_gpu(x, wp)
     N, D, H, W = x.shape[:4]
     sc = scratch(x.device) if stats is not None else None
+    desc = _defer_on(stats, defer and k == 3)
+    if desc is not None:
+        _ck(lib().msseg_conv3d_stem_fwd_deferred(_p(x), ld(x), _p(wp), _p(bias), _p(y), ld(y) if y is not None else 0, N, D,
+                                                 H, W, cout, _p(stats), _p(sc), sc.numel(), dt(x), C.addressof(desc),
+                                                 _stream()), "conv3d_stem_fwd_deferred")
+        return y
     fn = lib().msseg_conv3d_stem_fwd if k == 3 else lib().msseg_conv3d_stem_k1_fwd
     _ck(fn(_p(x), ld(x), _p(wp), _p(bias), _p(y), ld(y) if y is not None else 0, N, D, H, W, cout, _p(stats), _p(sc),
                                     sc.numel() if sc is not None else 0, dt(x), _stream()), "conv3d_stem_fwd")
@@ -909,9 +961,10 @@
 def instnorm_act_fwd(x, stats, gamma, beta, y, slope, eps=1e-5, residual=None):
     _need_gpu(x, stats, y)
     N, S, Cc = _nsc(x)
-    TIMER.launch("instnorm_act_fwd", 0.0, _nbytes(x, y, residual), lambda: _ck(lib().msseg_instnorm_act_fwd(_p(x), ld(x), _p(stats), _p(gamma), _p(beta), _p(residual),
+    desc, dp = _take_fin(stats)
+    TIMER.launch("instnorm_act_fwd", 0.0, _nbytes(x, y, residual), lambda: _ck(lib().msseg_instnorm_act_fwd_deferred(_p(x), ld(x), _p(stats), _p(gamma), _p(beta), _p(residual),
                                      ld(residual) if residual is not None else 0, _p(y), ld(y), N, S, Cc, eps, slope,
-                                     dt(x), _stream()), "instnorm_act_fwd"))
+                                     dt(x), dp, _stream()), "instnorm_act_fwd"))
     return y
 
 
@@ -924,8 +977,9 @@
 def instnorm_act_pool_fwd(x, stats, gamma, beta, y, pooled, slope, eps=1e-5):
     _need_gpu(x, stats, y, pooled)
     N, D, H, W, Cc = x.shape
-    TIMER.launch("instnorm_act_pool_fwd", 0.0, _nbytes(x, y, pooled), lambda: _ck(lib().msseg_instnorm_act_pool_fwd(_p(x), ld(x), _p(stats), _p(gamma), _p(beta), _p(y), ld(y), _p(pooled), ld(pooled),
-                                          N, D, H, W, Cc, eps, slope, dt(x), _stream()), "instnorm_act_pool_fwd"))
+    desc, dp = _take_fin(stats)
+    TIMER.launch("instnorm_act_pool_fwd", 0.0, _nbytes(x, y, pooled), lambda: _ck(lib().msseg_instnorm_act_pool_fwd_deferred(_p(x), ld(x), _p(stats), _p(gamma), _p(beta), _p(y), ld(y), _p(pooled), ld(pooled),
+                                          N, D, H, W, Cc, eps, slope, dt(x), dp, _stream()), "instnorm_act_pool_fwd"))
     return y, pooled
 
 
@@ -965,10 +1019,11 @@
 def instnorm_act_bwd_apply(x, stats, gamma, y, dy, red, dx, slope, eps=1e-5, dres=None, beta=None):
     _need_gpu(x, stats, dy, dx, red)
     N, S, Cc = _nsc(x)
-    TIMER.launch("instnorm_act_bwd_apply", 0.0, _nbytes(x, y, dy, dx, dres), lambda: _ck(lib().msseg_instnorm_act_bwd_apply(_p(x), ld(x), _p(stats), _p(gamma), _p(beta), _p(y),
+    desc, dp = _take_fin(red)
+    TIMER.launch("instnorm_act_bwd_apply", 0.0, _nbytes(x, y, dy, dx, dres), lambda: _ck(lib().msseg_instnorm_act_bwd_apply_deferred(_p(x), ld(x), _p(stats), _p(gamma), _p(beta), _p(y),
                                            ld(y) if y is not None else 0, _p(dy), ld(dy), _p(red),
                                            _p(dx), ld(dx), _p(dres), ld(dres) if dres is not None else 0, N, S, Cc, eps,
-                                           slope, dt(x), _stream()), "instnorm_act_bwd_apply"))
+                                           slope, dt(x), dp, _stream()), "instnorm_act_bwd_apply"))
     return red
 
 
diff --git a/medicalsemseg_amd/layers.py b/medicalsemseg_amd/layers.py
--- a/medicalsemseg_amd/layers.py
+++ b/medicalsemseg_amd/layers.py
@@ -214,7 +214,7 @@
     def _gather(self, dtype):
         return self.cin % (8 if dtype == torch.bfloat16 else 4) != 0
 
-    def fwd(self, x, out=None, want_stats=False):
+    def fwd(self, x, out=None, want_stats=False, defer_stats=False):
         dtype = x.dtype
         if want_stats and out is None and self.halves_ok(tuple(x.shape[:4]), dtype):
             return self.fwd_halves(x)
@@ -226,7 +226,7 @@
                     and not os.environ.get("MSSEG_NO_STEM")):
                 if want_stats and x.shape[0] <= 8:
                     stats = torch.empty(x.shape[0], self.cout, 2, dtype=torch.float32, device=x.device)
-                hip.conv3d_stem(x, wp, self.b, y, self.cout, stats)
+                hip.conv3d_stem(x, wp, self.b, y, self.cout, stats, defer=defer_stats)
             else:
                 hip.conv3d_gather(x, wp, self.b, y, self.cin, self.cout, 3, 1, 1)
         else:
@@ -234,7 +234,7 @@
             wp = self.cache.get(self.w, dtype, ("f", vol), lambda: hip.pack_conv_k3(self.w.detach(), dtype, vol=vol))
             if want_stats and x.shape[0] <= 8:
                 stats = torch.empty(x.shape[0], self.cout, 2, dtype=torch.float32, device=x.device)
-            hip.conv3d_k3(x, wp, self.b, y, self.cin, self.cout, stats)
+            hip.conv3d_k3(x, wp, self.b, y, self.cin, self.cout, stats, defer=defer_stats)
         if want_stats:
             return y, (stats if stats is not None else hip.channel_stats(y))
         return y
@@ -288,7 +288,8 @@
         vol = tuple(dy.shape[:4])
         return hip.lib().msseg_conv3d_k3_kernel(*vol, self.cout, self.cin, hip.BF16) == (4 if self.cout == 48 else 3)
 
-    def bwd(self, x, dy, need_dx=True, dx_out=None, bias_grad_is_zero=False, next_norm=None, accumulate_dx=False):
+    def bwd(self, x, dy, need_dx=True, dx_out=None, bias_grad_is_zero=False, next_norm=None, accumulate_dx=False,
+            defer_red=False):
         dtype = x.dtype
         if self.w.requires_grad:
             g, acc = _grad_buf(self.w)
@@ -339,7 +340,7 @@
                     dg, acc = _grad_buf(nrm.gamma)
                     db, _ = _grad_buf(nrm.beta)
                 red = hip.conv3d_k3_dgrad_inbwd(dy, wp, dx, self.cout, self.cin, yraw, act, stats, nrm.slope, nrm.eps,
-                                                dg, db, acc)
+                                                dg, db, acc, defer=defer_red)
                 return dx, red
             hip.conv3d_k3(dy, wp, None, dx, self.cout, self.cin)
             return dx, None
@@ -603,7 +604,7 @@
             stats = torch.empty(x.shape[0], cv.cout, 2, dtype=torch.float32, device=x.device)
             hip.conv3d_k3_small_fwd_finish(part, ng, cv.b, nm.gamma, nm.beta, nm.eps, nm.slope, y, a, pooled, stats)
             return a, (x, y, stats, a)
-        y, stats = self.conv.fwd(x, want_stats=True)
+        y, stats = self.conv.fwd(x, want_stats=True, defer_stats=True)
         a, stats = self.norm.fwd(y, out, stats=stats, pooled=pooled)
         return a, (x, y, stats, a)
 
@@ -612,7 +613,8 @@
         dy = self.norm.bwd(y, stats, a, da, red=red)
         if next_cna is not None and need_dx:
             nx, ny, nstats, na = next_saved
-            return self.conv.bwd(x, dy, True, bias_grad_is_zero=True, next_norm=(next_cna.norm, ny, nstats, na))
+            return self.conv.bwd(x, dy, True, bias_grad_is_zero=True, next_norm=(next_cna.norm, ny, nstats, na),
+                                 defer_red=True)
         return self.conv.bwd(x, dy, need_dx, bias_grad_is_zero=True)
 
 
```
